# protolambda/go-kzg

Hardware: AMD Instinct MI355X
Metric: KZG commitments/sec (CommitToPoly, 4096-element blob); FK20 half: value_fk20_4096 (higher is better)
Workload: dtype u32; 1 GPU; CommitToPoly, 4096-coeff blobs, eth/trusted_setup.json monomial setup (s=1337), 4096 blobs/step/GPU resident in HBM, fixed-base table budget 110 GB (library default 110 GB: signed 16-bit windows, 8 of them walked by both GLV halves of every scalar, 103 GB; see table_sweep); global_batch=4096, parallelism=dp1 (independent blobs, no data-path collective)

## Files before the change

### go-kzg_amd/csrc/capi_common.hpp

```cpp
#pragma once
#include "../../include/kzg_hip.h"
#include "kzg_hip_internal.h"
#include "internal.hpp"
#include "fr_fft4096.hpp"
#include "fr_das2048.hpp"
#include "coalesce.hpp"
#include "sha256.hpp"

#include <algorithm>
#include <atomic>
#include <map>
#include <memory>
#include <mutex>
#include <shared_mutex>
#include <new>
#include <string>
#include <thread>
#include <chrono>
#include <condition_variable>
#include <vector>
#include <cstdio>
#include <cstring>
#include <cstdlib>

using namespace kzg;

extern thread_local std::string g_last_error;

#define HIPCHK(expr)                                                                                         \
    do {                                                                                                     \
        hipError_t e_ = (expr);                                                                              \
        if (e_ != hipSuccess) {                                                                              \
            char buf_[512];                                                                                  \
            snprintf(buf_, sizeof buf_, "%s failed: %s (%s:%d)", #expr, hipGetErrorString(e_), __FILE__, __LINE__); \
            g_last_error = buf_;                                                                             \
            (void)hipGetLastError();  \
            return KZG_HIP_ERR_HIP;                                                                          \
        }                                                                                                    \
    } while (0)
#define CHK(expr) do { int s_ = (expr); if (s_ != KZG_HIP_OK) return s_; } while (0)
#define KZG_TRY try {
#define KZG_CATCH                                                                                             \
    } catch (const std::bad_alloc &) { g_last_error = "host allocation failed"; return KZG_HIP_ERR_HIP; }    \
    catch (const std::exception &e_) { g_last_error = e_.what(); return KZG_HIP_ERR_HIP; }

inline bool is_pow2(uint64_t v) { return (v & (v - 1)) == 0; }
inline uint64_t next_pow2(uint64_t v) { if (v == 0) return 1; uint64_t p = 1; while (p < v) p <<= 1; return p; }

struct kzg_hip_fft {
    int device = 0;
    hipStream_t stream = nullptr;
    unsigned max_scale = 0;
    uint64_t W = 0;
    std::vector<fr> h_expanded, h_reversed;
    fr *d_expanded = nullptr, *d_reversed = nullptr;
    fr *d_expanded_l = nullptr, *d_reversed_l = nullptr;
    fr *d_inv_pow2 = nullptr;
    uint32_t *d_tw_das2048 = nullptr;
    uint32_t *d_tw4096[2] = {nullptr, nullptr};
    fr *d_glv_expanded = nullptr, *d_glv_reversed = nullptr;
    int8_t *d_wnaf_expanded = nullptr, *d_wnaf_reversed = nullptr;
    uint8_t *h_stage = nullptr; size_t h_stage_cap = 0;
    std::mutex mu;
    struct pool_slot { hipStream_t s = nullptr; uint8_t *h_pin = nullptr; size_t pin_cap = 0; };
    std::mutex pool_mu; std::condition_variable pool_cv; std::vector<pool_slot> pool_idle; int pool_total = 0;
    g2a *d_g2_fb = nullptr; uint64_t g2_fb_builds = 0;
    struct lincomb_promo *promo = nullptr;
};
struct g2_state;
struct kzg_hip_kzg {
    kzg_hip_fft *fs = nullptr;
    uint64_t n_setup = 0;
    g1j *d_secret = nullptr;
    g1a *d_secret_a = nullptr;
    g1a *d_fixed = nullptr;
    msm_plan fixed_plan{};
    double budget_gb = -1.0;
    std::atomic<bool> projective{false};
    hipStream_t copy_stream = nullptr;
    hipEvent_t copy_done[2] = {nullptr, nullptr};
    std::unique_ptr<coalescer> co_commit, co_proof;
    std::shared_ptr<g2_state> g2;
    std::mutex g2_mu;
    std::shared_mutex tab_mu;
};
struct fk20_core {
    kzg_hip_kzg *ks = nullptr;
    uint64_t n2 = 0, l = 1, k = 0;
    g1j *d_files = nullptr;
    g1a *d_files_fb = nullptr;
    uint32_t fb_c = 0, fb_nwin = 0; bool fb_glv = false;
    std::unique_ptr<coalescer> co_da;
};
struct kzg_hip_fk20s { fk20_core c; };
struct kzg_hip_fk20m { fk20_core c; };

struct dev_guard {
    kzg_hip_fft *fs; std::unique_lock<std::mutex> lk;
    explicit dev_guard(kzg_hip_fft *f) : fs(f), lk(f->mu) { hipSetDevice(f->device); }
};

struct dev_select { explicit dev_select(kzg_hip_fft *f) { hipSetDevice(f->device); } };
struct stream_lease {
    static constexpr int POOL_MAX = 16;
    static constexpr size_t PIN_MAX = 8u << 20;
    kzg_hip_fft *fs; hipStream_t s = nullptr; kzg_hip_fft::pool_slot slot; std::unique_lock<std::mutex> fallback;
    explicit stream_lease(kzg_hip_fft *f) : fs(f) {
        hipSetDevice(f->device);
        std::unique_lock<std::mutex> lk(f->pool_mu);
        for (;;) {
            if (!f->pool_idle.empty()) { slot = f->pool_idle.back(); f->pool_idle.pop_back(); s = slot.s; return; }
            if (f->pool_total < POOL_MAX) {
                if (hipStreamCreateWithFlags(&slot.s, hipStreamNonBlocking) == hipSuccess) { stream_cache_own(slot.s); f->pool_total++; s = slot.s; return; }
                (void)hipGetLastError(); slot.s = nullptr;
                if (f->pool_total == 0) { lk.unlock(); fallback = std::unique_lock<std::mutex>(f->mu); s = f->stream; return; }
            }
            f->pool_cv.wait(lk);
        }
    }
    stream_lease(kzg_hip_fft *f, std::try_to_lock_t) : fs(f) {
        std::unique_lock<std::mutex> lk(f->pool_mu);
        if (!f->pool_idle.empty()) { slot = f->pool_idle.back(); f->pool_idle.pop_back(); s = slot.s; return; }
        if (f->pool_total >= POOL_MAX) return;
        if (hipStreamCreateWithFlags(&slot.s, hipStreamNonBlocking) == hipSuccess) { stream_cache_own(slot.s); f->pool_total++; s = slot.s; return; }
        (void)hipGetLastError(); slot.s = nullptr;
    }
    uint8_t *pinned(size_t bytes, void **dev) {
        if (fallback.owns_lock() || bytes > PIN_MAX) return nullptr;
        if (slot.pin_cap < bytes) {
            if (slot.h_pin) { hipHostFree(slot.h_pin); slot.h_pin = nullptr; slot.pin_cap = 0; }
            size_t cap = bytes < (1u << 20) ? (1u << 20) : bytes;
            if (hipHostMalloc((void **)&slot.h_pin, cap, hipHostMallocDefault) != hipSuccess) { (void)hipGetLastError(); slot.h_pin = nullptr; return nullptr; }
            slot.pin_cap = cap;
        }
        if (hipHostGetDevicePointer(dev, slot.h_pin, 0) != hipSuccess) { (void)hipGetLastError(); return nullptr; }
        return slot.h_pin;
    }
    ~stream_lease() {
        if (!s) return;
        if (fallback.owns_lock()) { (void)hipStreamSynchronize(s); return; }
        (void)hipStreamSynchronize(slot.s);
        std::lock_guard<std::mutex> lk(fs->pool_mu);
        fs->pool_idle.push_back(slot);
        fs->pool_cv.notify_one();
    }
};
inline int d2h_staged(kzg_hip_fft *fs, hipStream_t s, void *host_dst, const void *dev_src, size_t bytes) {
    if (bytes > (16u << 20) || bytes < (1u << 20)) {
        HIPCHK(hipMemcpyAsync(host_dst, dev_src, bytes, hipMemcpyDeviceToHost, s));
        HIPCHK(hipStreamSynchronize(s));
        return KZG_HIP_OK;
    }
    if (fs->h_stage_cap < bytes) {
        if (fs->h_stage) { hipHostFree(fs->h_stage); fs->h_stage = nullptr; fs->h_stage_cap = 0; }
        size_t cap = 8u << 20;
        while (cap < bytes) cap <<= 1;
        if (hipHostMalloc((void **)&fs->h_stage, cap, hipHostMallocDefault) != hipSuccess) {
            (void)hipGetLastError(); fs->h_stage = nullptr;
            HIPCHK(hipMemcpyAsync(host_dst, dev_src, bytes, hipMemcpyDeviceToHost, s));
            HIPCHK(hipStreamSynchronize(s));
            return KZG_HIP_OK;
        }
        fs->h_stage_cap = cap;
    }
    HIPCHK(hipMemcpyAsync(fs->h_stage, dev_src, bytes, hipMemcpyDeviceToHost, s));
    HIPCHK(hipStreamSynchronize(s));
    memcpy(host_dst, fs->h_stage, bytes);
    return KZG_HIP_OK;
}
struct drain_on_exit {
    hipStream_t s;
    explicit drain_on_exit(hipStream_t st) : s(st) {}
    ~drain_on_exit() { (void)hipStreamSynchronize(s); }
};
void stream_cache_own(hipStream_t s);
void stream_cache_disown(hipStream_t s);
void *stream_cache_take(hipStream_t s, size_t class_bytes);
bool stream_cache_give(hipStream_t s, void *p, size_t class_bytes);
inline size_t stream_cache_class(size_t bytes) {
    if (bytes > (8u << 20)) return 0;
    size_t c = 256;
    while (c < bytes) c <<= 1;
    return c;
}
template <class T> struct dtmp {
    T *p = nullptr; hipStream_t s; size_t cls = 0;
    dtmp(hipStream_t st) : s(st) {}
    int alloc(size_t count) {
        if (!count) count = 1;
        size_t bytes = count * sizeof(T);
        cls = stream_cache_class(bytes);
        if (cls) {
            if ((p = (T *)stream_cache_take(s, cls))) return KZG_HIP_OK;
            bytes = cls;
        }
        HIPCHK(hipMallocAsync((void **)&p, bytes, s));
        return KZG_HIP_OK;
    }
    ~dtmp() { if (p && !(cls && stream_cache_give(s, p, cls))) hipFreeAsync(p, s); }
};


struct kzg_hip_points {
    kzg_hip_fft *fs = nullptr;
    uint64_t n = 0;
    g1a *d_tab = nullptr;
    kzg_hip_kzg *ks = nullptr;
    std::unique_ptr<coalescer> co;
};
struct kzg_hip_eth {
    kzg_hip_fft *fs = nullptr;
    kzg_hip_kzg *ks = nullptr;
    uint64_t n = 0;
    fr *d_domain = nullptr;
    std::unique_ptr<coalescer> co_blob;
    std::unique_ptr<coalescer> co_proof;
    std::shared_ptr<g2_state> g2;
    std::mutex g2_mu;
    std::vector<std::pair<hipEvent_t, std::shared_ptr<g2_state>>> g2_queued;
};

void fr_fft_rows(kzg_hip_fft *fs, hipStream_t s, const fr *d_in, uint64_t in_stride, uint64_t n_in, fr *d_out, uint64_t n, uint64_t batch, int inv);
uint32_t g1_fft_direct_logr(uint64_t n, uint64_t batch);
bool g1_fft_direct_mode(uint64_t n, uint64_t batch);
int g1_fft_direct_lanes(uint64_t n, uint64_t batch);
int g1_fft_rows(kzg_hip_fft *fs, hipStream_t s, const g1j *d_in, uint64_t in_stride, uint64_t n_valid, g1j *d_data, uint64_t n, uint64_t batch, int inv,
                           const fr *scale = nullptr, uint64_t n_out = 0);
int das_ext_rows(kzg_hip_fft *fs, hipStream_t s, fr *d, uint64_t n, uint64_t batch);
msm_plan classic_plan(uint64_t n, bool folded = false);
void set_inf_image(void *out_g1);
int kzg_settings_build(kzg_hip_fft *fs, const void *points_g1, uint64_t n, kzg_hip_kzg **out);
int ensure_fixed_table(kzg_hip_kzg *ks, hipStream_t);
const void *host_mapped_pointer(const void *host, size_t bytes);
int h2d_copy(void *dst, const void *src, size_t bytes, hipStream_t s);
int commit_rows(kzg_hip_kzg *ks, hipStream_t s, const fr *d_sc, uint64_t n, uint64_t batch, g1j *d_out, uint64_t sc_stride = 0, bool to_kilic = true);
double table_budget_gb(knobs::opt_gb env, double cap_gb, double headroom_gb);
int lincomb_points_rows(kzg_hip_points *pts, hipStream_t s, const fr *d_sc, uint64_t n, uint64_t batch, g1j *d_out, uint64_t sc_stride = 0, bool holds_mu = false);
int lincomb_points_coalesced(kzg_hip_points *pts, const void *scalars_fr, uint64_t n, void *out_g1);
uint32_t fb_windows(uint32_t c);
uint32_t fb_windows_glv(uint32_t c);
bool fb_glv_enabled();
bool coalescing_enabled();
coalescer *get_coalescer(kzg_hip_fft *fs, std::unique_ptr<coalescer> &slot, size_t in_row, size_t out_row, int callers_per_batch = 0);
int coalesce_upload_rows(coalesce_buf &b, uint64_t batch, size_t in_row_bytes, uint64_t n_max, fr *d_rows, uint64_t *d_meta);
int proof_single_rows(kzg_hip_kzg *ks, hipStream_t s, const fr *d_poly, uint64_t n, uint64_t batch, const uint64_t *d_x_u64, uint64_t x_stride, g1j *d_out);
int eth_g2_lines(kzg_hip_eth *eth, std::shared_ptr<g2_state> &hold, const g2_prepared **gen, const g2_prepared **s1);
int eth_g2_hold_on_stream(kzg_hip_eth *eth, hipStream_t s, const std::shared_ptr<g2_state> &hold);
void eth_g2_release_passed(kzg_hip_eth *eth, bool all = false);
int fk20_hext(fk20_core *c, hipStream_t s, const fr *d_poly, uint64_t poly_stride, uint64_t n, uint64_t batch, uint64_t j0, uint64_t cnt, g1j *d_hext);
int fk20_finish(fk20_core *c, hipStream_t s, const g1j *d_hext, uint64_t batch, int da, int bit_reverse, g1j *d_out);
int fk20_run_dev(fk20_core *c, hipStream_t s, const fr *d_poly, uint64_t poly_stride, uint64_t n, uint64_t batch, int da, int bit_reverse, g1j *d_out);
```

### go-kzg_amd/csrc/capi_kzg.hip

```cpp
#include "capi_common.hpp"

int kzg_settings_build(kzg_hip_fft *fs, const void *points_g1, uint64_t n, kzg_hip_kzg **out) {
    dev_guard g(fs);
    hipStream_t s = fs->stream;
    std::unique_ptr<kzg_hip_kzg, void (*)(kzg_hip_kzg *)> own(new kzg_hip_kzg, kzg_hip_kzg_settings_free);
    kzg_hip_kzg *ks = own.get();
    ks->fs = fs; ks->n_setup = n;
    dtmp<g1j> d_raw(s);
    CHK(d_raw.alloc(n));
    HIPCHK(hipMalloc((void **)&ks->d_secret, n * sizeof(g1j)));
    HIPCHK(hipMalloc((void **)&ks->d_secret_a, n * sizeof(g1a)));
    HIPCHK(hipMemcpyAsync(d_raw.p, points_g1, n * sizeof(g1j), hipMemcpyHostToDevice, s));
    launch_g1_from_kilic(s, d_raw.p, n);
    launch_g1_normalize(s, d_raw.p, ks->d_secret, n);
    launch_g1_to_affine(s, ks->d_secret, ks->d_secret_a, n);
    HIPCHK(hipGetLastError());
    HIPCHK(hipStreamSynchronize(s));
    *out = own.release();
    return KZG_HIP_OK;
}
int kzg_hip_kzg_settings_new(kzg_hip_fft *fs, const void *secret_g1, uint64_t n_setup, kzg_hip_kzg **out) {
    if (!fs || !out || !secret_g1) return KZG_HIP_ERR_BAD_ARG;
    *out = nullptr;
    if (n_setup < fs->W) return KZG_HIP_ERR_LEN_MISMATCH;
    KZG_TRY
    return kzg_settings_build(fs, secret_g1, n_setup, out);
    KZG_CATCH
}
void kzg_hip_kzg_settings_free(kzg_hip_kzg *ks) {
    if (!ks) return;
    hipSetDevice(ks->fs->device);
    hipDeviceSynchronize();
    hipFree(ks->d_secret); hipFree(ks->d_secret_a); hipFree(ks->d_fixed);
    if (ks->copy_stream) { stream_cache_disown(ks->copy_stream); hipStreamDestroy(ks->copy_stream); }
    for (int i = 0; i < 2; i++) if (ks->copy_done[i]) hipEventDestroy(ks->copy_done[i]);
    (void)hipGetLastError();
    delete ks;
}

double table_budget_gb(knobs::opt_gb env, double cap_gb, double headroom_gb) {
    if (env.set) return env.gb;
    size_t free_b = 0, total_b = 0;
    if (hipMemGetInfo(&free_b, &total_b) != hipSuccess) return 0.0;
    double g = (double)free_b / 1e9 - headroom_gb;
    return g > cap_gb ? cap_gb : (g > 0.0 ? g : 0.0);
}
uint32_t fb_windows(uint32_t c) {
    uint32_t nw = (255 + c - 1) / c, sh = c * (nw - 1);
    uint64_t top = (0x73eda753299d7d48ull >> (sh - 192)) + 1;
    return top > (1ull << (c - 1)) ? nw + 1 : nw;
}

#ifndef FB_DEFAULT_BUDGET_GB
#define FB_DEFAULT_BUDGET_GB 110.0
#endif
uint32_t fb_windows_glv(uint32_t c) { return (128 + c - 1) / c; }
bool fb_glv_enabled() { return knobs::fb_glv(); }
int ensure_fixed_table(kzg_hip_kzg *ks, hipStream_t) {
    if (ks->d_fixed || ks->fixed_plan.c == 0xffffffffu) return KZG_HIP_OK;
    hipStream_t s = ks->fs->stream;
    double budget_gb = ks->budget_gb >= 0.0 ? ks->budget_gb : table_budget_gb(knobs::fb_budget_gb(), FB_DEFAULT_BUDGET_GB, 24.0);
    if (ks->n_setup < 64) { ks->fixed_plan.c = 0xffffffffu; return KZG_HIP_OK; }
    const bool glv = fb_glv_enabled();
    for (uint32_t c = 16; c >= 5; c--) {
        if (glv ? (c == 14) : (c == 15)) continue;
        const uint32_t nwin = glv ? fb_windows_glv(c) : fb_windows(c);
        double bytes = (double)nwin * (double)ks->n_setup * (double)(1u << (c - 1)) * sizeof(g1a);
        if (bytes > budget_gb * 1e9) continue;
        msm_plan p{};
        p.c = c; p.nwin = nwin; p.nb = 1u << (c - 1); p.ngroups = 1; p.fixed = 1; p.glv = glv ? 1 : 0; p.table_n = ks->n_setup;
        size_t entries = (size_t)p.nwin * ks->n_setup * p.nb;
        g1a *tab = nullptr;
        if (hipMalloc((void **)&tab, entries * sizeof(g1a)) != hipSuccess) { (void)hipGetLastError(); continue; }
        hipError_t e = launch_fb_build(s, ks->d_secret_a, ks->n_setup, p.c, p.nwin, tab);
        if (e == hipSuccess) e = hipStreamSynchronize(s);
        if (e != hipSuccess) { (void)hipGetLastError(); hipFree(tab); continue; }
        ks->d_fixed = tab; ks->fixed_plan = p;
        return KZG_HIP_OK;
    }
    ks->fixed_plan.c = 0xffffffffu;
    return KZG_HIP_OK;
}

int commit_rows(kzg_hip_kzg *ks, hipStream_t s, const fr *d_sc, uint64_t n, uint64_t batch, g1j *d_out, uint64_t sc_stride, bool to_kilic) {
    CHK(ensure_fixed_table(ks, s));
    bool fixed = ks->d_fixed != nullptr;
    if (!sc_stride) sc_stride = n;
    msm_plan p = fixed ? ks->fixed_plan : classic_plan(ks->n_setup);
    if (!fixed && !msm_index_range_ok(p, n)) return KZG_HIP_ERR_TOO_WIDE;
    size_t ws_main = fixed ? fb_partials_bytes(n, batch) : msm_workspace_bytes(p, n, batch);
    dtmp<uint8_t> d_ws(s);
    CHK(d_ws.alloc(ws_main));
    if (fixed) launch_fb_msm(s, ks->d_fixed, p.table_n, p.c, p.nwin, d_sc, sc_stride, n, batch, d_ws.p, d_out, to_kilic, p.glv != 0, to_kilic && ks->projective.load(std::memory_order_relaxed));
    else launch_msm(s, p, ks->d_secret_a, d_sc, sc_stride, n, batch, d_ws.p, d_out, to_kilic);
    HIPCHK(hipGetLastError());
    return KZG_HIP_OK;
}
int kzg_hip_kzg_set_table_budget_gb(kzg_hip_kzg *ks, double gb) {
    if (!ks || !(gb >= 0.0)) return KZG_HIP_ERR_BAD_ARG;
    std::unique_lock<std::shared_mutex> tl(ks->tab_mu);
    dev_guard g(ks->fs);
    if (ks->d_fixed) { HIPCHK(hipDeviceSynchronize()); HIPCHK(hipFree(ks->d_fixed)); ks->d_fixed = nullptr; }
    ks->fixed_plan = msm_plan{};
    ks->budget_gb = gb;
    return KZG_HIP_OK;
}

int kzg_hip_commit_to_poly_batch_dev(kzg_hip_kzg *ks, const void *d_coeffs_fr, uint64_t n, uint64_t batch, void *d_out_g1, void *stream) {
    if (!ks || !d_out_g1) return KZG_HIP_ERR_BAD_ARG;
    if (n > ks->n_setup) return KZG_HIP_ERR_LEN_MISMATCH;
    if (!batch) return KZG_HIP_OK;
    if (n == 0 || !d_coeffs_fr) return KZG_HIP_ERR_BAD_ARG;
    dev_guard g(ks->fs);
    return commit_rows(ks, (hipStream_t)stream, (const fr *)d_coeffs_fr, n, batch, (g1j *)d_out_g1);
}
namespace {
std::mutex g_reg_mu;
std::map<uintptr_t, size_t> g_registered;
}
const void *host_mapped_pointer(const void *host, size_t bytes) {
    hipPointerAttribute_t a;
    if (hipPointerGetAttributes(&a, host) != hipSuccess) { (void)hipGetLastError(); return nullptr; }
    if (a.type != hipMemoryTypeHost || !a.devicePointer) return nullptr;
    const uintptr_t h = (uintptr_t)host;
    {
        std::lock_guard<std::mutex> lk(g_reg_mu);
        auto it = g_registered.upper_bound(h);
        if (it != g_registered.begin()) {
            --it;
            if (h >= it->first && h < it->first + it->second) return (h + bytes <= it->first + it->second) ? a.devicePointer : nullptr;
        }
    }
    hipDeviceptr_t base = nullptr; size_t size = 0;
    if (hipMemGetAddressRange(&base, &size, (hipDeviceptr_t)a.devicePointer) != hipSuccess) { (void)hipGetLastError(); return nullptr; }
    const uintptr_t d = (uintptr_t)a.devicePointer, b = (uintptr_t)base;
    return (d >= b && d + bytes <= b + size) ? a.devicePointer : nullptr;
}
int h2d_copy(void *dst, const void *src, size_t bytes, hipStream_t s) {
    uintptr_t p = (uintptr_t)src; uint8_t *d = (uint8_t *)dst;
    while (bytes) {
        size_t chunk = bytes;
        {
            std::lock_guard<std::mutex> lk(g_reg_mu);
            auto it = g_registered.upper_bound(p);
            if (it != g_registered.end() && it->first - p < chunk) chunk = it->first - p;
            if (it != g_registered.begin()) {
                --it;
                if (p < it->first + it->second && it->first + it->second - p < chunk) chunk = it->first + it->second - p;
            }
        }
        HIPCHK(hipMemcpyAsync(d, (const void *)p, chunk, hipMemcpyHostToDevice, s));
        p += chunk; d += chunk; bytes -= chunk;
    }
    return KZG_HIP_OK;
}
int kzg_hip_host_register(void *host, uint64_t bytes) {
    if (!host || !bytes) return KZG_HIP_ERR_BAD_ARG;
    KZG_TRY
    {
        std::lock_guard<std::mutex> lk(g_reg_mu);
        const uintptr_t h = (uintptr_t)host;
        auto it = g_registered.lower_bound(h);
        if (it != g_registered.end() && it->first < h + bytes) { g_last_error = "kzg_hip_host_register: the range overlaps a registered one (unregister it first)"; return KZG_HIP_ERR_BAD_ARG; }
        if (it != g_registered.begin()) { --it; if (it->first + it->second > h) { g_last_error = "kzg_hip_host_register: the range overlaps a registered one (unregister it first)"; return KZG_HIP_ERR_BAD_ARG; } }
    }
    HIPCHK(hipHostRegister(host, bytes, hipHostRegisterPortable | hipHostRegisterMapped));
    std::lock_guard<std::mutex> lk(g_reg_mu);
    g_registered[(uintptr_t)host] = bytes;
    return KZG_HIP_OK;
    KZG_CATCH
}
int kzg_hip_host_unregister(void *host) {
    if (!host) return KZG_HIP_ERR_BAD_ARG;
    KZG_TRY
    {
        std::lock_guard<std::mutex> lk(g_reg_mu);
        const uintptr_t h = (uintptr_t)host;
        auto it = g_registered.upper_bound(h);
        if (it != g_registered.begin()) {
            --it;
            if (h > it->first && h < it->first + it->second) { g_last_error = "kzg_hip_host_unregister: the address lies inside a registered range but is not its base"; return KZG_HIP_ERR_BAD_ARG; }
        }
    }
    HIPCHK(hipHostUnregister(host));
    std::lock_guard<std::mutex> lk(g_reg_mu);
    g_registered.erase((uintptr_t)host);
    return KZG_HIP_OK;
    KZG_CATCH
}
int kzg_hip_commit_to_poly_batch(kzg_hip_kzg *ks, const void *coeffs_fr, uint64_t n, uint64_t batch, void *out_g1) {
    if (!ks || !out_g1) return KZG_HIP_ERR_BAD_ARG;
    if (n > ks->n_setup) return KZG_HIP_ERR_LEN_MISMATCH;
    if (!batch) return KZG_HIP_OK;
    if (n == 0) { for (uint64_t b = 0; b < batch; b++) set_inf_image((uint8_t *)out_g1 + b * sizeof(g1j)); return KZG_HIP_OK; }
    if (!coeffs_fr) return KZG_HIP_ERR_BAD_ARG;
    dev_guard g(ks->fs);
    hipStream_t s = ks->fs->stream;
    dtmp<fr> d_sc(s); dtmp<g1j> d_out(s);
    CHK(d_out.alloc(batch));
    if (const fr *mapped = (const fr *)host_mapped_pointer(coeffs_fr, (size_t)n * batch * sizeof(fr))) {
        CHK(commit_rows(ks, s, mapped, n, batch, d_out.p));
        HIPCHK(hipMemcpyAsync(out_g1, d_out.p, batch * sizeof(g1j), hipMemcpyDeviceToHost, s));
        HIPCHK(hipStreamSynchronize(s));
        return KZG_HIP_OK;
    }
    CHK(d_sc.alloc(n * batch));
    uint64_t chunk = batch >= 1024 ? 512 : (batch >= 512 ? 256 : batch);
    if (chunk < batch && n * sizeof(fr) >= (64u << 10)) {
        if (!ks->copy_stream) {
            HIPCHK(hipStreamCreateWithFlags(&ks->copy_stream, hipStreamNonBlocking));
            stream_cache_own(ks->copy_stream);
            for (int i = 0; i < 2; i++) HIPCHK(hipEventCreateWithFlags(&ks->copy_done[i], hipEventDisableTiming));
        }
        CHK(ensure_fixed_table(ks, s));
        HIPCHK(hipStreamSynchronize(s));
        const bool ramp = knobs::upload_ramp() && batch >= 1024;
        int slot = 0;
        uint64_t step = 0;
        for (uint64_t b0 = 0, cnt = 0; b0 < batch; b0 += cnt, slot ^= 1, step++) {
            uint64_t want = chunk;
            if (ramp && step == 0) want = 64; else if (ramp && step == 1) want = 192;
            cnt = batch - b0 < want ? batch - b0 : want;
            CHK(h2d_copy(d_sc.p + b0 * n, (const fr *)coeffs_fr + b0 * n, n * cnt * sizeof(fr), ks->copy_stream));
            HIPCHK(hipEventRecord(ks->copy_done[slot], ks->copy_stream));
            HIPCHK(hipStreamWaitEvent(s, ks->copy_done[slot], 0));
            CHK(commit_rows(ks, s, d_sc.p + b0 * n, n, cnt, d_out.p + b0));
        }
    } else {
        CHK(h2d_copy(d_sc.p, coeffs_fr, n * batch * sizeof(fr), s));
        CHK(commit_rows(ks, s, d_sc.p, n, batch, d_out.p));
    }
    HIPCHK(hipMemcpyAsync(out_g1, d_out.p, batch * sizeof(g1j), hipMemcpyDeviceToHost, s));
    HIPCHK(hipStreamSynchronize(s));
    return KZG_HIP_OK;
}
bool coalescing_enabled() { return knobs::coalesce(); }
static uint64_t coalesce_rows(size_t in_row, size_t out_row) {
    size_t row = in_row > out_row ? in_row : out_row;
    uint64_t r = (64u << 20) / (row ? row : 1);
    return r < 4 ? 4 : (r > 256 ? 256 : r);
}
coalescer *get_coalescer(kzg_hip_fft *fs, std::unique_ptr<coalescer> &slot, size_t in_row, size_t out_row, int callers_per_batch) {
    std::lock_guard<std::mutex> lk(fs->mu);
    if (!slot) slot.reset(new coalescer(fs->device, in_row, out_row, coalesce_rows(in_row, out_row), callers_per_batch));
    return slot.get();
}
int coalesce_upload_rows(coalesce_buf &b, uint64_t batch, size_t in_row_bytes, uint64_t n_max, fr *d_rows, uint64_t *d_meta) {
    hipStream_t s = b.stream;
    HIPCHK(hipMemcpyAsync(d_meta, b.h_meta, batch * sizeof(coalesce_row), hipMemcpyHostToDevice, s));
    if (in_row_bytes == n_max * sizeof(fr)) HIPCHK(hipMemcpyAsync(d_rows, b.h_in, batch * in_row_bytes, hipMemcpyHostToDevice, s));
    else if (batch <= 4) { for (uint64_t r = 0; r < batch; r++) HIPCHK(hipMemcpyAsync(d_rows + r * n_max, b.h_in + r * in_row_bytes, n_max * sizeof(fr), hipMemcpyHostToDevice, s)); }
    else HIPCHK(hipMemcpy2DAsync(d_rows, n_max * sizeof(fr), b.h_in, in_row_bytes, n_max * sizeof(fr), batch, hipMemcpyHostToDevice, s));
    launch_fr_zero_tails(s, d_rows, n_max, batch, d_meta, 2);
    return KZG_HIP_OK;
}
int kzg_hip_commit_to_poly(kzg_hip_kzg *ks, const void *coeffs_fr, uint64_t n, void *out_g1) {
    if (!coalescing_enabled() || !ks || !out_g1 || !coeffs_fr || n == 0 || n > ks->n_setup)
        return kzg_hip_commit_to_poly_batch(ks, coeffs_fr, n, 1, out_g1);
    KZG_TRY
    coalescer *co = get_coalescer(ks->fs, ks->co_commit, ks->n_setup * sizeof(fr), sizeof(g1j));
    auto exec = [ks, co](coalesce_buf &b, uint64_t batch) -> int {
        hipSetDevice(ks->fs->device);
        hipStream_t s = b.stream;
        drain_on_exit drain(s);
        std::shared_lock<std::shared_mutex> tl(ks->tab_mu);
        { dev_guard g(ks->fs); CHK(ensure_fixed_table(ks, s)); }
        uint64_t n_max = 0;
        for (uint64_t i = 0; i < batch; i++) n_max = b.h_meta[i].n > n_max ? b.h_meta[i].n : n_max;
        dtmp<fr> d_rows(s); dtmp<uint64_t> d_meta(s);
        void *dp_out = nullptr;
        HIPCHK(hipHostGetDevicePointer(&dp_out, b.h_out, 0));
        g1j *d_out = (g1j *)dp_out;
        const bool trace = knobs::coalesce_trace();
        const auto t0 = std::chrono::steady_clock::now();
        bool uniform = ks->d_fixed != nullptr;
        for (uint64_t i = 0; i < batch && uniform; i++) uniform = b.h_meta[i].n == n_max;
        const fr *d_src = d_rows.p; uint64_t stride = n_max;
        if (uniform) {
            void *dp = nullptr;
            HIPCHK(hipHostGetDevicePointer(&dp, b.h_in, 0));
            d_src = (const fr *)dp; stride = co->in_row_bytes() / sizeof(fr);
        } else {
            CHK(d_rows.alloc(batch * n_max)); CHK(d_meta.alloc(2 * batch));
            d_src = d_rows.p;
            CHK(coalesce_upload_rows(b, batch, co->in_row_bytes(), n_max, d_rows.p, d_meta.p));
        }
        if (trace) hipStreamSynchronize(s);
        const auto t1 = std::chrono::steady_clock::now();
        CHK(commit_rows(ks, s, d_src, n_max, batch, d_out, stride));
        if (trace) hipStreamSynchronize(s);
        const auto t2 = std::chrono::steady_clock::now();
        HIPCHK(hipStreamSynchronize(s));
        if (trace) {
            auto us = [](std::chrono::steady_clock::time_point a, std::chrono::steady_clock::time_point c) { return std::chrono::duration<double, std::micro>(c - a).count(); };
            fprintf(stderr, "[commit batch %llu] upload %.0f us, kernels %.0f us, final synchronisation %.0f us\n", (unsigned long long)batch, us(t0, t1), us(t1, t2),
                    us(t2, std::chrono::steady_clock::now()));
        }
        return KZG_HIP_OK;
    };
    return co->submit(coeffs_fr, n * sizeof(fr), n, 0, out_g1, sizeof(g1j), exec, KZG_HIP_ERR_HIP);
    KZG_CATCH
}

int lincomb_points_coalesced(kzg_hip_points *pts, const void *scalars_fr, uint64_t n, void *out_g1) {
    if (!coalescing_enabled()) return kzg_hip_lincomb_points_batch(pts, scalars_fr, n, 1, out_g1);
    KZG_TRY
    coalescer *co = get_coalescer(pts->fs, pts->co, pts->n * sizeof(fr), sizeof(g1j));
    auto exec = [pts, co](coalesce_buf &b, uint64_t batch) -> int {
        hipSetDevice(pts->fs->device);
        hipStream_t s = b.stream;
        drain_on_exit drain(s);
        uint64_t n_max = 0;
        for (uint64_t i = 0; i < batch; i++) n_max = b.h_meta[i].n > n_max ? b.h_meta[i].n : n_max;
        bool uniform = true;
        for (uint64_t i = 0; i < batch && uniform; i++) uniform = b.h_meta[i].n == n_max;
        dtmp<fr> d_rows(s); dtmp<uint64_t> d_meta(s);
        void *dp_out = nullptr;
        HIPCHK(hipHostGetDevicePointer(&dp_out, b.h_out, 0));
        const fr *d_src; uint64_t stride;
        if (uniform) {
            void *dp = nullptr;
            HIPCHK(hipHostGetDevicePointer(&dp, b.h_in, 0));
            d_src = (const fr *)dp; stride = co->in_row_bytes() / sizeof(fr);
        } else {
            CHK(d_rows.alloc(batch * n_max)); CHK(d_meta.alloc(2 * batch));
            CHK(coalesce_upload_rows(b, batch, co->in_row_bytes(), n_max, d_rows.p, d_meta.p));
            d_src = d_rows.p; stride = n_max;
        }
        CHK(lincomb_points_rows(pts, s, d_src, n_max, batch, (g1j *)dp_out, stride));
        HIPCHK(hipStreamSynchronize(s));
        return KZG_HIP_OK;
    };
    return co->submit(scalars_fr, n * sizeof(fr), n, 0, out_g1, sizeof(g1j), exec, KZG_HIP_ERR_HIP);
    KZG_CATCH
}

int proof_single_rows(kzg_hip_kzg *ks, hipStream_t s, const fr *d_poly, uint64_t n, uint64_t batch, const uint64_t *d_x_u64, uint64_t x_stride, g1j *d_out) {
    dtmp<fr> d_q(s), d_x(s);
    CHK(d_q.alloc(batch * (n - 1))); CHK(d_x.alloc(batch));
    launch_fr_from_u64(s, d_x_u64, x_stride, d_x.p, batch);
    launch_quotient_linear(s, d_poly, n, n, batch, d_x.p, d_q.p, n - 1);
    return commit_rows(ks, s, d_q.p, n - 1, batch, d_out);
}
int kzg_hip_compute_proof_single_batch_dev(kzg_hip_kzg *ks, const void *d_poly_fr, uint64_t n, uint64_t batch, const void *d_x_u64, void *d_out_g1, void *stream) {
    if (!ks || !d_out_g1 || n < 2) return KZG_HIP_ERR_BAD_ARG;
    if (n - 1 > ks->n_setup) return KZG_HIP_ERR_LEN_MISMATCH;
    if (!batch) return KZG_HIP_OK;
    if (!d_poly_fr || !d_x_u64) return KZG_HIP_ERR_BAD_ARG;
    dev_guard g(ks->fs);
    return proof_single_rows(ks, (hipStream_t)stream, (const fr *)d_poly_fr, n, batch, (const uint64_t *)d_x_u64, 1, (g1j *)d_out_g1);
}
int kzg_hip_compute_proof_single_batch(kzg_hip_kzg *ks, const void *poly_fr, uint64_t n, uint64_t batch, const uint64_t *xs, void *out_g1) {
    if (!ks || !out_g1 || n < 2) return KZG_HIP_ERR_BAD_ARG;
    if (n - 1 > ks->n_setup) return KZG_HIP_ERR_LEN_MISMATCH;
    if (!batch) return KZG_HIP_OK;
    if (!poly_fr || !xs) return KZG_HIP_ERR_BAD_ARG;
    dev_guard g(ks->fs);
    hipStream_t s = ks->fs->stream;
    dtmp<fr> d_poly(s); dtmp<uint64_t> d_x(s); dtmp<g1j> d_out(s);
    CHK(d_poly.alloc(n * batch)); CHK(d_x.alloc(batch)); CHK(d_out.alloc(batch));
    HIPCHK(hipMemcpyAsync(d_poly.p, poly_fr, n * batch * sizeof(fr), hipMemcpyHostToDevice, s));
    HIPCHK(hipMemcpyAsync(d_x.p, xs, batch * sizeof(uint64_t), hipMemcpyHostToDevice, s));
    CHK(proof_single_rows(ks, s, d_poly.p, n, batch, d_x.p, 1, d_out.p));
    HIPCHK(hipMemcpyAsync(out_g1, d_out.p, batch * sizeof(g1j), hipMemcpyDeviceToHost, s));
    HIPCHK(hipStreamSynchronize(s));
    return KZG_HIP_OK;
}
int kzg_hip_compute_proof_single(kzg_hip_kzg *ks, const void *poly_fr, uint64_t n, uint64_t x, void *out_g1) {
    if (!ks || !poly_fr || !out_g1 || n < 2) return KZG_HIP_ERR_BAD_ARG;
    if (!coalescing_enabled() || n - 1 > ks->n_setup) return kzg_hip_compute_proof_single_batch(ks, poly_fr, n, 1, &x, out_g1);
    KZG_TRY
    coalescer *co = get_coalescer(ks->fs, ks->co_proof, (ks->n_setup + 1) * sizeof(fr), sizeof(g1j));
    auto exec = [ks, co](coalesce_buf &b, uint64_t batch) -> int {
        hipSetDevice(ks->fs->device);
        hipStream_t s = b.stream;
        drain_on_exit drain(s);
        std::shared_lock<std::shared_mutex> tl(ks->tab_mu);
        { dev_guard g(ks->fs); CHK(ensure_fixed_table(ks, s)); }
        uint64_t n_max = 0;
        for (uint64_t i = 0; i < batch; i++) n_max = b.h_meta[i].n > n_max ? b.h_meta[i].n : n_max;
        void *dp_out = nullptr;
        HIPCHK(hipHostGetDevicePointer(&dp_out, b.h_out, 0));
        if (batch == 1) {
            void *dp_in = nullptr, *dp_meta = nullptr;
            HIPCHK(hipHostGetDevicePointer(&dp_in, b.h_in, 0));
            HIPCHK(hipHostGetDevicePointer(&dp_meta, b.h_meta, 0));
            CHK(proof_single_rows(ks, s, (const fr *)dp_in, n_max, 1, (const uint64_t *)dp_meta + 1, 2, (g1j *)dp_out));
            HIPCHK(hipStreamSynchronize(s));
            return KZG_HIP_OK;
        }
        dtmp<fr> d_rows(s); dtmp<uint64_t> d_meta(s);
        CHK(d_rows.alloc(batch * n_max)); CHK(d_meta.alloc(2 * batch));
        CHK(coalesce_upload_rows(b, batch, co->in_row_bytes(), n_max, d_rows.p, d_meta.p));
        CHK(proof_single_rows(ks, s, d_rows.p, n_max, batch, d_meta.p + 1, 2, (g1j *)dp_out));
        HIPCHK(hipStreamSynchronize(s));
        return KZG_HIP_OK;
    };
    return co->submit(poly_fr, n * sizeof(fr), n, x, out_g1, sizeof(g1j), exec, KZG_HIP_ERR_HIP);
    KZG_CATCH
}

int kzg_hip_compute_proof_multi(kzg_hip_kzg *ks, const void *poly_fr, uint64_t len, uint64_t x, uint64_t n, void *out_g1) {
    (void)x;
    if (!ks || !poly_fr || !out_g1 || len < n + 1) return KZG_HIP_ERR_BAD_ARG;
    uint64_t nq = len - n;
    if (nq > ks->n_setup) return KZG_HIP_ERR_LEN_MISMATCH;
    return kzg_hip_commit_to_poly(ks, (const uint8_t *)poly_fr + n * sizeof(fr), nq, out_g1);
}
int kzg_hip_check_proof_multi_interpolation(kzg_hip_kzg *ks, const void *ys_fr, uint64_t n, const void *x_fr, void *out_is1_g1, void *out_xpow_fr) {
    if (!ks || !ys_fr || !x_fr || !out_is1_g1 || n == 0) return KZG_HIP_ERR_BAD_ARG;
    kzg_hip_fft *fs = ks->fs;
    if (n > fs->W) return KZG_HIP_ERR_TOO_WIDE;
    uint64_t np = next_pow2(n);
    if (np > ks->n_setup) return KZG_HIP_ERR_LEN_MISMATCH;
    dev_guard g(fs);
    hipStream_t s = fs->stream;
    dtmp<fr> d_ys(s), d_ip(s), d_x(s); dtmp<g1j> d_out(s);
    CHK(d_ys.alloc(n)); CHK(d_ip.alloc(np)); CHK(d_x.alloc(2)); CHK(d_out.alloc(1));
    HIPCHK(hipMemcpyAsync(d_ys.p, ys_fr, n * sizeof(fr), hipMemcpyHostToDevice, s));
    HIPCHK(hipMemcpyAsync(d_x.p, x_fr, sizeof(fr), hipMemcpyHostToDevice, s));
    fr_fft_rows(fs, s, d_ys.p, n, n, d_ip.p, np, 1, 1);
    launch_fr_scale_by_inv_powers(s, d_ip.p, d_x.p, np, d_x.p + 1);
    CHK(commit_rows(ks, s, d_ip.p, np, 1, d_out.p));
    HIPCHK(hipMemcpyAsync(out_is1_g1, d_out.p, sizeof(g1j), hipMemcpyDeviceToHost, s));
    if (out_xpow_fr) HIPCHK(hipMemcpyAsync(out_xpow_fr, d_x.p + 1, sizeof(fr), hipMemcpyDeviceToHost, s));
    HIPCHK(hipStreamSynchronize(s));
    return KZG_HIP_OK;
}
int kzg_hip_toeplitz_part2(kzg_hip_kzg *ks, const void *coeffs_fr, const void *x_ext_fft_g1, uint64_t n, void *out_g1) {
    if (!ks || !coeffs_fr || !x_ext_fft_g1 || !out_g1) return KZG_HIP_ERR_BAD_ARG;
    kzg_hip_fft *fs = ks->fs;
    if (n > fs->W) return KZG_HIP_ERR_TOO_WIDE;
    if (!is_pow2(n) || n == 0) return KZG_HIP_ERR_LEN_MISMATCH;
    stream_lease lease(fs);
    hipStream_t s = lease.s;
    dtmp<fr> d_c(s), d_cf(s); dtmp<g1j> d_x(s), d_h(s);
    CHK(d_c.alloc(n)); CHK(d_cf.alloc(n)); CHK(d_x.alloc(n)); CHK(d_h.alloc(n));
    HIPCHK(hipMemcpyAsync(d_c.p, coeffs_fr, n * sizeof(fr), hipMemcpyHostToDevice, s));
    HIPCHK(hipMemcpyAsync(d_x.p, x_ext_fft_g1, n * sizeof(g1j), hipMemcpyHostToDevice, s));
    launch_g1_from_kilic(s, d_x.p, n);
    fr_fft_rows(fs, s, d_c.p, n, n, d_cf.p, n, 1, 0);
    launch_g1_mul_vec(s, d_x.p, n, d_cf.p, 1, n, d_h.p);
    launch_g1_normalize(s, d_h.p, d_x.p, n, true);
    HIPCHK(hipGetLastError());
    HIPCHK(hipMemcpyAsync(out_g1, d_x.p, n * sizeof(g1j), hipMemcpyDeviceToHost, s));
    HIPCHK(hipStreamSynchronize(s));
    return KZG_HIP_OK;
}
int kzg_hip_toeplitz_part3(kzg_hip_kzg *ks, const void *h_ext_fft_g1, uint64_t n, void *out_g1) {
    if (!ks) return KZG_HIP_ERR_BAD_ARG;
    if (n > ks->fs->W) return KZG_HIP_ERR_TOO_WIDE;
    if (!is_pow2(n)) return KZG_HIP_ERR_NOT_POW2;
    if (n == 0 || !h_ext_fft_g1 || !out_g1) return KZG_HIP_ERR_BAD_ARG;
    KZG_TRY
    std::vector<g1j> full(n);
    CHK(kzg_hip_fft_g1(ks->fs, h_ext_fft_g1, n, 1, full.data()));
    memcpy(out_g1, full.data(), (n / 2) * sizeof(g1j));
    return KZG_HIP_OK;
    KZG_CATCH
}

int kzg_hip_kzg_table_info(kzg_hip_kzg *ks, uint32_t *window_bits, uint32_t *windows, uint64_t *table_bytes) {
    if (!ks || !window_bits || !windows || !table_bytes) return KZG_HIP_ERR_BAD_ARG;
    bool have = ks->d_fixed != nullptr;
    *window_bits = have ? ks->fixed_plan.c : 0; *windows = have ? ks->fixed_plan.nwin : 0;
    *table_bytes = have ? (uint64_t)ks->fixed_plan.nwin * ks->fixed_plan.table_n * ks->fixed_plan.nb * sizeof(g1a) : 0;
    return KZG_HIP_OK;
}
int kzg_hip_kzg_set_projective_outputs(kzg_hip_kzg *ks, int on) {
    if (!ks) return KZG_HIP_ERR_BAD_ARG;
    ks->projective.store(on != 0, std::memory_order_relaxed);
    return KZG_HIP_OK;
}
uint32_t kzg_hip_kzg_table_additions(kzg_hip_kzg *ks) {
    if (!ks || !ks->d_fixed) return 0;
    return ks->fixed_plan.glv ? 2 * ks->fixed_plan.nwin : ks->fixed_plan.nwin;
}
```

### go-kzg_amd/csrc/internal.hpp

```cpp
#pragma once
#include <hip/hip_runtime.h>
#include <stdint.h>
#include "field.hpp"
#include "g1.hpp"
#include "knobs.hpp"

namespace kzg {

inline uint32_t ilog2(uint64_t v) { uint32_t r = 0; while ((1ull << r) < v) r++; return r; }

void launch_fr_fft(hipStream_t s, const fr *in, uint64_t in_stride, uint64_t n_in, fr *out, uint64_t n, uint64_t batch,
                   const fr *roots, uint64_t W, const fr *scale, const uint32_t *tw4096 = nullptr, const fr *roots_l = nullptr);
bool fr_fft_lazy_sizes(uint64_t n, uint64_t batch);
void launch_das_ext(hipStream_t s, fr *vals, uint64_t n, uint64_t batch, const fr *expanded, const fr *reversed, uint64_t W,
                    const fr *inv_n, const uint32_t *tw2048 = nullptr);
void launch_toeplitz_coeffs(hipStream_t s, const fr *poly, uint64_t poly_stride, uint64_t n, uint64_t l, uint64_t batch, fr *out,
                            const fr *scale);
void launch_quotient_linear(hipStream_t s, const fr *poly, uint64_t poly_stride, uint64_t n, uint64_t batch, const fr *x, fr *q, uint64_t q_stride);
void launch_fr_from_u64(hipStream_t s, const uint64_t *in, uint64_t in_stride, fr *out, uint64_t n);
void launch_fr_zero_tails(hipStream_t s, fr *rows, uint64_t n_max, uint64_t batch, const uint64_t *lens, uint64_t lens_stride);
void launch_fr_any_nonzero(hipStream_t s, const fr *vals, uint64_t n, uint32_t *flag);
void launch_fr_powers(hipStream_t s, const fr *base, uint64_t n, fr *out);

void launch_fr_from_le32(hipStream_t s, const uint8_t *in, fr *out, uint64_t per_blob, uint64_t batch, uint32_t *bad);
void launch_fr_to_le32(hipStream_t s, const fr *in, uint8_t *out, uint64_t n);
void launch_fr_bitrev_gather(hipStream_t s, const fr *in, fr *out, uint64_t n);
constexpr uint64_t ZERO_TREE_LEAF = 16;
void launch_zero_leaves(hipStream_t s, const fr *expanded, uint64_t stride, const uint64_t *missing, uint64_t n_missing, uint64_t leaves, fr *a);
void launch_zero_pair_products(hipStream_t s, const fr *f, uint64_t m, uint64_t pairs, fr *out);
void launch_zero_join(hipStream_t s, fr *c, const fr *a, uint64_t d, uint64_t pairs);
void launch_zero_unpad(hipStream_t s, const fr *root, uint64_t pad, uint64_t n_missing, uint64_t length, fr *poly);
void launch_fr_mul_table_rows(hipStream_t s, fr *data, const fr *table, uint64_t stride, uint64_t n, uint64_t batch);
void launch_poly_lincomb(hipStream_t s, const fr *vectors, uint64_t stride, const fr *scalars, uint64_t count, uint64_t n, fr *out);
void launch_eth_quotient(hipStream_t s, const fr *poly, uint64_t poly_stride, const fr *domain, uint64_t n, uint64_t batch, const fr *z, uint64_t z_stride,
                         const fr *inv_n, fr *q, fr *y_out, uint32_t *flag, uint64_t dom_stride = 1, fr *scratch = nullptr);
uint64_t eth_quotient_scratch_elems(uint64_t n, uint64_t batch);

void launch_fr_scale_by_inv_powers(hipStream_t s, fr *c, const fr *x, uint64_t n, fr *xpow_n);

void launch_zero_eval_direct(hipStream_t s, const fr *expanded, uint64_t stride, const uint64_t *missing, uint64_t n_missing, uint64_t length, fr *zero_eval);
void launch_fr_scale_by_powers(hipStream_t s, fr *poly, const fr *base, uint64_t n);
void launch_fr_pointwise(hipStream_t s, const fr *a, const fr *b, const uint8_t *present, fr *out, uint64_t n, int mode, uint32_t *flag);
uint32_t launch_zero_eval_direct_rows_segs(uint64_t length, uint64_t rows, uint64_t nm_hint);
void launch_zero_eval_direct_rows(hipStream_t s, const fr *expanded, uint64_t stride, const uint64_t *missing, uint64_t list_stride, const uint64_t *n_missing, const fr *corr,
                                  uint32_t segs, uint64_t length, uint64_t rows, fr *zero_eval);

void launch_rr_scan(hipStream_t s, const uint8_t *present, uint64_t n, uint64_t rows, uint64_t *list, uint32_t *count, uint64_t *nm);
void launch_rr_corr(hipStream_t s, const uint64_t *nm, uint64_t rows, uint32_t segs, fr *corr);
void launch_rr_shift_bases(hipStream_t s, const fr &inv5, const fr &five, fr *out);
void launch_rr_leaves(hipStream_t s, const fr *expanded, uint64_t stride, const uint64_t *list, uint64_t list_stride, const uint64_t *nm, uint64_t leaves, uint64_t rows, fr *a);
void launch_rr_unpad(hipStream_t s, const fr *root, uint64_t leaves, const uint64_t *nm, uint64_t length, uint64_t rows, fr *poly);
void launch_rr_mask_mul(hipStream_t s, const fr *a, const fr *b, uint64_t b_stride, const uint8_t *present, uint64_t p_stride, uint64_t n, uint64_t rows, fr *out);
void launch_rr_strip_divide(hipStream_t s, const fr *num, const fr *den, fr *out, uint64_t total);
void launch_rr_finish(hipStream_t s, const fr *recon, const fr *samples, const uint8_t *present, uint64_t p_stride, const uint32_t *count, uint64_t c_stride, uint32_t *flag,
                      uint64_t n, uint64_t rows, fr *out, uint8_t *status);

void launch_g1_mul_vec(hipStream_t s, const g1j *pts, uint64_t pts_mod, const fr *scalars, uint64_t s_stride, uint64_t n, g1j *out);
hipError_t launch_g1_file_msm(hipStream_t s, const g1j *files, const fr *scalars, uint64_t nfiles, uint64_t k2, uint64_t j0, uint64_t cnt,
                              uint64_t batch, g1j *out);
void launch_g1_bitrev_copy(hipStream_t s, const g1j *in, uint64_t in_stride, uint64_t n_valid, g1j *out, uint64_t n, uint64_t batch);
void launch_g1_fft_stage(hipStream_t s, g1j *data, uint64_t n, uint64_t batch, uint64_t m, const fr *roots, const int8_t *wnaf, uint64_t W);
struct g1_stage_plan { int lanes; bool wnaf; bool rows; };
g1_stage_plan g1_fft_stage_plan(uint64_t n, uint64_t batch, uint64_t m, bool dif, int quad, knobs::g1_mul_mode mul);
g1_stage_plan g1_fft_stage_plan(uint64_t n, uint64_t batch, uint64_t m, bool dif);
void launch_g1_fft_stage_planned(hipStream_t s, const g1_stage_plan &plan, bool dif, g1j *data, uint64_t n, uint64_t batch, uint64_t m, const fr *roots, const int8_t *wnaf, uint64_t W);
void launch_g1_fft_stage_dif(hipStream_t s, g1j *data, uint64_t n, uint64_t batch, uint64_t m, const fr *roots, const int8_t *wnaf, uint64_t W);
void launch_g1_clear_odd(hipStream_t s, g1j *data, uint64_t n_total);
void launch_g1_take_even(hipStream_t s, const g1j *in, g1j *out, uint64_t total);
bool g1_quad_enabled();
void launch_fb_direct_pass1(hipStream_t s, const g1a *table, uint64_t table_n, uint32_t c, uint32_t nwin, const fr *scalars, const fr *roots, uint64_t W, uint64_t batch,
                            uint32_t logR, g1j *out, bool glv = false);
void launch_g1_stage_coop_dif(hipStream_t s, int lanes, bool wnaf_rows, g1j *data, uint64_t n, uint64_t batch, uint64_t m, const fr *roots, const int8_t *wnaf, uint64_t W, uint64_t total);
void launch_g1_stage_coop_dit(hipStream_t s, int lanes, bool wnaf_rows, g1j *data, uint64_t n, uint64_t batch, uint64_t m, const fr *roots, const int8_t *wnaf, uint64_t W, uint64_t total);
void launch_g1_direct_coop(hipStream_t s, int lanes, uint32_t wgs, size_t pad_lds, const g1j *src, uint64_t src_stride, uint64_t src_valid, g1j *dst, uint32_t logn, uint32_t logR,
                           uint64_t Ns, const fr *roots, uint64_t W, const fr *sc, uint64_t total, uint32_t logT, uint32_t logU);
void launch_g1_fft_direct(hipStream_t s, const g1j *in, uint64_t in_stride, uint64_t n_valid, g1j *data, g1j *tmp, uint64_t n, uint64_t batch, const fr *roots,
                          uint64_t W, const fr *scale, uint32_t max_logr = 4, int lanes = 1, uint32_t bits_done = 0, uint64_t n_out = 0,
                          bool lanes_fixed = false);
void launch_g1_normalize(hipStream_t s, const g1j *in, g1j *out, uint64_t n, bool to_kilic = false);
void launch_fr_inv_test(hipStream_t s, const fr *in, uint64_t n, fr *out_coop, fr *out_lane, fr *out_block);
void launch_fp_inv_both(hipStream_t s, const fp *in, fp *out_coop, fp *out_lane, uint64_t n, int mode);
void launch_g1_from_kilic(hipStream_t s, g1j *data, uint64_t n);
void launch_g1_to_affine(hipStream_t s, const g1j *in, g1a *out, uint64_t n);
void launch_g1_compress(hipStream_t s, const g1j *in, uint8_t *out48, uint64_t n);
void launch_g1_decompress(hipStream_t s, const uint8_t *in48, g1j *out, uint64_t n, uint32_t *bad_flag);
void launch_g1_fixed_base_powers(hipStream_t s, const fr *powers, uint64_t n, g1j *out);

uint64_t device_simd_lanes();
inline uint64_t device_simds() { return device_simd_lanes() / 64; }
struct msm_plan {
    uint32_t c;
    uint32_t nwin;
    uint32_t nb;
    uint32_t ngroups;
    uint32_t fixed;
    uint32_t glv;
    uint64_t table_n;
};
inline bool msm_index_range_ok(const msm_plan &p, uint64_t n) { return n < (1ull << 27) && 2 * p.table_n < (1ull << 30); }
size_t msm_workspace_bytes(const msm_plan &p, uint64_t n, uint64_t batch);
void launch_msm(hipStream_t s, const msm_plan &p, const g1a *table, const fr *scalars, uint64_t sc_stride, uint64_t n, uint64_t batch, void *workspace, g1j *out,
                bool to_kilic, uint64_t table_stride = 0, bool crowded_buckets = false);
void launch_msm_window_table(hipStream_t s, const g1a *pts, uint64_t n, uint32_t c, uint32_t nwin, g1j *tmp, g1a *out);

size_t fb_partials_bytes(uint64_t n, uint64_t batch);
hipError_t launch_fb_build(hipStream_t s, const g1a *pts, uint64_t n, uint32_t c, uint32_t nwin, g1a *table);
void launch_fb_msm(hipStream_t s, const g1a *table, uint64_t table_n, uint32_t c, uint32_t nwin, const fr *scalars, uint64_t sc_stride, uint64_t n,
                   uint64_t batch, void *partials, g1j *out, bool to_kilic, bool glv = false, bool projective = false);

void launch_fb_mul_vec(hipStream_t s, const g1a *table, uint64_t table_n, uint32_t c, uint32_t nwin, const fr *scalars, uint64_t row, uint64_t j0,
                       uint64_t cnt, uint64_t batch, g1j *out, bool glv = false);
void launch_fb_mul_vec_dif2(hipStream_t s, const g1a *table, uint64_t table_n, uint32_t c, uint32_t nwin, const fr *scalars, const fr *roots, uint64_t W,
                            uint64_t batch, g1j *out, bool glv = false);
void launch_fb_mul_vec_files(hipStream_t s, const g1a *table, uint64_t table_n, uint32_t c, uint32_t nwin, const fr *scalars, uint64_t row, uint64_t j0,
                             uint64_t cnt, uint64_t batch, g1j *out, bool glv = false);
void launch_g1_sum_files(hipStream_t s, const g1j *tmp, uint64_t nfiles, uint64_t cnt, uint64_t batch, g1j *out);

struct g2j; struct g2_prepared;
void launch_g2_from_compressed(hipStream_t s, const uint8_t *in96, g2j *out_kilic, uint64_t n, uint32_t *bad_flag);
void launch_g2_prepare(hipStream_t s, const g2j *in_kilic, uint64_t n, g2_prepared *out);
void launch_pairs_g1_from_kilic(hipStream_t s, const g1j *a1, const g1j *b1, uint64_t n, g1j *p0, g1j *p1);
void launch_kzg_check_inputs(hipStream_t s, const g1j *c, const g1j *pi, const fr *ys, const g1j *es, const fr *bs, uint64_t n, g1j *p0, g1j *p1);
void launch_fr_rows_scale_by_inv_powers(hipStream_t s, fr *c, uint64_t np, const fr *xs, uint64_t count, fr *xpow_n);
void launch_eth_check_inputs(hipStream_t s, const uint8_t *c48, const uint8_t *zs, const uint8_t *ys, const uint8_t *pi48, uint64_t n, g1j *p0, g1j *p1, uint8_t *status);
void launch_pairing_check(hipStream_t s, bool shared_lines, const g2_prepared *q0, const g2_prepared *q1, const g1j *p0, const g1j *p1, uint64_t n, uint8_t *ok);
void launch_pairing_value(hipStream_t s, const g1j *g1_kilic, const g2_prepared *q, uint64_t n, fp *out);
bool pairing_route_is_wave(uint64_t n);

constexpr uint64_t PAIRING_WAVE_BELOW = 16385;
void launch_pairing_check_wave(hipStream_t s, bool shared_lines, const g2_prepared *q0, const g2_prepared *q1, const g1j *p0, const g1j *p1, uint64_t n, uint8_t *ok);
void launch_pairing_value_wave(hipStream_t s, const g1j *g1_kilic, const g2_prepared *q, uint64_t n, fp *out);
void launch_wave_fp12_op(hipStream_t s, int op, const fp *a, const fp *b, uint64_t n, fp *out);

struct g2a;
void launch_g2_fixed_base_table(hipStream_t s, g2a *table);
void launch_g2_fixed_base(hipStream_t s, const fr *scalars, uint64_t n, const g2a *table, g2j *out);
void launch_g2_normalize(hipStream_t s, const g2j *in, uint64_t n, g2j *out_kilic);
void launch_g2_compress(hipStream_t s, const g2j *in_kilic, uint64_t n, uint8_t *out96);

void launch_eth_transcripts(hipStream_t s, const uint8_t *blobs, const uint8_t *comms, const uint64_t *off, uint64_t n, uint64_t sidecars, fr *r_out, fr *z_out);
void launch_eth_transcript_blobs(hipStream_t s, const uint8_t *blobs, const uint64_t *off, uint64_t n, uint64_t sidecars, uint32_t *st);
void launch_eth_transcript_finish(hipStream_t s, const uint8_t *blobs, const uint8_t *comms, const uint64_t *off, uint64_t n, uint64_t sidecars, const uint32_t *st,
                                  fr *r_out, fr *z_out);
void launch_eth_prove_finish(hipStream_t s, const uint8_t *agg_status, const uint32_t *z_in_domain, const uint64_t *off, uint64_t sidecars, uint8_t code_blob,
                             uint8_t code_z, uint8_t *proofs48, uint8_t *comms48, uint8_t *status);
void launch_eth_agg_poly(hipStream_t s, const uint8_t *blobs, const uint64_t *off, const fr *r, uint64_t n, uint64_t sidecars, fr *agg, uint8_t *status);
void launch_eth_powers(hipStream_t s, const fr *r, const uint64_t *off, uint64_t sidecars, fr *pow);
void launch_g1_decompress_rows(hipStream_t s, const uint8_t *in48, g1j *out, uint64_t n, uint8_t *bad, bool to_kilic);
void launch_g1_segment_sum(hipStream_t s, const g1j *pts, const uint8_t *pt_bad, const uint64_t *off, uint64_t sidecars, g1j *out, g1j *out_kilic, uint8_t *status);
void launch_eth_agg_finish(hipStream_t s, const uint32_t *z_in_domain, const uint8_t *proof_bad, uint64_t sidecars, fr *y, uint8_t *status);
void launch_test_sha256_lanes(hipStream_t s, const uint8_t *data, const uint64_t *offsets, const uint64_t *lens, uint64_t rows, uint32_t *out);
void launch_test_hash_to_bls_field_lanes(hipStream_t s, const uint8_t *digests, uint64_t rows, fr *out);

void launch_eth_versioned_hashes(hipStream_t s, const uint8_t *c48, uint64_t n, uint8_t *out32);
void launch_eth_precompile_inputs(hipStream_t s, const uint8_t *in192, uint64_t n, g1j *p0, g1j *p1, uint8_t *status);
void launch_eth_merge_status(hipStream_t s, const uint8_t *status, const uint8_t *ok, uint64_t n, uint8_t *result);
void launch_eth_tx_hashes_check(hipStream_t s, const uint8_t *c48, const uint8_t *want32, const uint64_t *off, uint64_t total, uint64_t blocks, uint8_t *match,
                                uint8_t *result);

struct combine_seed;
void launch_combine_scalars(hipStream_t s, const combine_seed &seed, const fr *xs, const fr *ys, const uint8_t *status, uint64_t row0, uint64_t count, uint64_t R, fr *sc);
void launch_combine_points(hipStream_t s, const g1j *c, const g1j *pi, uint64_t count, uint64_t R, bool kilic, g1j *out, const g1j *last = nullptr);
void launch_combine_negate(hipStream_t s, const g1j *a, uint64_t n, g1j *out);
void launch_eth_combine_fields(hipStream_t s, const uint8_t *zs, const uint8_t *ys, const uint8_t *c_bad, const uint8_t *pi_bad, uint64_t n, fr *z_out, fr *y_out,
                               uint8_t *status);

void launch_combine_multi_scalars(hipStream_t s, const combine_seed &seed, const fr *xs, const fr *coef, uint64_t np, uint64_t row0, uint64_t count, uint64_t R, fr *sc,
                                  fr *partials, fr *J);

void prof_begin(hipStream_t s, const char *name);
void prof_end(hipStream_t s, const char *name);

}
```

### go-kzg_amd/csrc/k_msm.hip

```cpp
#include "internal.hpp"
#include "g1_quad.hpp"
#include "coop_inv.hpp"
#include <atomic>
#include <cstring>

namespace kzg {

#define MSM_SORT_T 1024
#define MSM_ACC_BLOCK 128
#define MSM_NB 128

struct fb_partial { uint32_t w[52]; uint32_t inf; };
__device__ __forceinline__ void fb_partial_store(fb_partial &o, const g1x_acc &a) {
#pragma unroll
    for (int i = 0; i < 13; i++) { o.w[i] = a.v.x.l[i]; o.w[13 + i] = a.v.y.l[i]; o.w[26 + i] = a.v.zz.l[i]; o.w[39 + i] = a.v.zzz.l[i]; }
    o.inf = a.inf ? 1u : 0u;
}
__device__ __forceinline__ void fb_partial_load(const fb_partial &p, g1xq &v) {
#pragma unroll
    for (int i = 0; i < 13; i++) { v.x.l[i] = p.w[i]; v.y.l[i] = p.w[13 + i]; v.zz.l[i] = p.w[26 + i]; v.zzz.l[i] = p.w[39 + i]; }
}

template <uint32_t DELTA> __device__ __forceinline__ uint32_t lane_down(uint32_t v) {
    if constexpr (DELTA < 16) return (uint32_t)__builtin_amdgcn_update_dpp((int)v, (int)v, 0x100 + DELTA, 0xf, 0xf, false);
    else return (uint32_t)__builtin_amdgcn_ds_bpermute((int)((((threadIdx.x & 63u) + DELTA) & 63u) << 2), (int)v);
}
template <uint32_t DELTA> __device__ __forceinline__ void point_down(g1xq &o, uint32_t &oinf, const g1xq &v, uint32_t vinf) {
#pragma unroll
    for (int i = 0; i < 13; i++) {
        o.x.l[i] = lane_down<DELTA>(v.x.l[i]); o.y.l[i] = lane_down<DELTA>(v.y.l[i]);
        o.zz.l[i] = lane_down<DELTA>(v.zz.l[i]); o.zzz.l[i] = lane_down<DELTA>(v.zzz.l[i]);
    }
    oinf = lane_down<DELTA>(vinf);
}
__device__ __forceinline__ void point_down_any(g1xq &o, uint32_t &oinf, const g1xq &v, uint32_t vinf, uint32_t off) {
    switch (off) {
    case 4: point_down<4>(o, oinf, v, vinf); break;
    case 8: point_down<8>(o, oinf, v, vinf); break;
    case 16: point_down<16>(o, oinf, v, vinf); break;
    default: point_down<32>(o, oinf, v, vinf); break;
    }
}

#ifndef MSM_SEG
#define MSM_SEG 64
#endif
struct msm_ws_layout {
    size_t entries_off, offsets_off, buckets_off, gsum_off, segs_off, per_blob;
    uint64_t K, nent, nseg;
};
static msm_ws_layout ws_layout(const msm_plan &p, uint64_t n) {
    msm_ws_layout L;
    L.K = (uint64_t)p.ngroups * MSM_NB;
    L.nent = n * 32;
    size_t o = 0;
    L.entries_off = o; o += ((L.nent * 4 + 15) / 16) * 16;
    L.offsets_off = o; o += (((2 * L.K + 1) * 4 + 15) / 16) * 16;
    L.buckets_off = o; o += ((L.K * sizeof(fb_partial) + 15) / 16) * 16;
    L.gsum_off = o; o += (((size_t)p.ngroups * sizeof(fb_partial) + 15) / 16) * 16;
    L.nseg = (L.nent + MSM_SEG - 1) / MSM_SEG;
    L.segs_off = o; o += ((L.nseg * 2 * sizeof(fb_partial) + 15) / 16) * 16;
    L.per_blob = o;
    return L;
}
size_t msm_workspace_bytes(const msm_plan &p, uint64_t n, uint64_t batch) { return ws_layout(p, n).per_blob * batch; }

template <class Fn> __device__ __forceinline__ void for_each_glv_digit(const fr &k_mont, Fn f) {
    const glv_halves h = glv_split_signed(from_mont<FrP>(k_mont));
#pragma unroll
    for (uint32_t half = 0; half < 2; half++) {
        const uint32_t *mag = half ? h.k2 : h.k1;
        const uint32_t sgn = half ? h.neg2 : h.neg1;
        uint32_t carry = 0;
#pragma unroll
        for (uint32_t w = 0; w < 16; w++) {
            uint32_t raw = ((mag[w >> 2] >> ((w & 3) * 8)) & 255u) + carry;
            if (raw > MSM_NB) { carry = 1; f(w, 256u - raw, half, sgn ^ 1u); }
            else { carry = 0; f(w, raw, half, sgn); }
        }
    }
}

__global__ __launch_bounds__(MSM_SORT_T) void k_msm_sort(uint32_t ngroups, uint64_t table_n, const fr *scalars, uint64_t sc_stride, uint64_t n, uint8_t *ws,
                                                         size_t per_blob, size_t entries_off, size_t offsets_off, uint32_t K) {
    extern __shared__ uint32_t smem[];
    uint32_t *hist = smem, *part = smem + K;
    const uint32_t tid = threadIdx.x;
    const uint64_t b = blockIdx.x;
    const fr *sc = scalars + b * sc_stride;
    uint32_t *entries = (uint32_t *)(ws + b * per_blob + entries_off);
    uint32_t *offsets = (uint32_t *)(ws + b * per_blob + offsets_off);
    const uint32_t wmask = ngroups - 1;
    for (uint32_t i = tid; i < K; i += MSM_SORT_T) hist[i] = 0;
    __syncthreads();
    for (uint64_t i = tid; i < n; i += MSM_SORT_T)
        for_each_glv_digit(sc[i], [&](uint32_t w, uint32_t mag, uint32_t half, uint32_t) {
            if (mag) atomicAdd(&hist[(((w & wmask) * MSM_NB + mag - 1) << 1) | (half ^ 1u)], 1u);
        });
    __syncthreads();
    const uint32_t per = (K + MSM_SORT_T - 1) / MSM_SORT_T;
    uint32_t lo = tid * per, hi = lo + per < K ? lo + per : K, sum = 0;
    for (uint32_t i = lo; i < hi; i++) sum += hist[i];
    part[tid] = sum;
    __syncthreads();
    for (uint32_t off = 1; off < MSM_SORT_T; off <<= 1) {
        uint32_t v = tid >= off ? part[tid - off] : 0;
        __syncthreads();
        part[tid] += v;
        __syncthreads();
    }
    uint32_t run = part[tid] - sum;
    for (uint32_t i = lo; i < hi; i++) { uint32_t cnt = hist[i]; offsets[i] = run; hist[i] = run; run += cnt; }
    if (tid == MSM_SORT_T - 1) offsets[K] = part[tid];
    __syncthreads();
    for (uint64_t i = tid; i < n; i += MSM_SORT_T)
        for_each_glv_digit(sc[i], [&](uint32_t w, uint32_t mag, uint32_t half, uint32_t neg) {
            if (!mag) return;
            uint32_t slot = atomicAdd(&hist[(((w & wmask) * MSM_NB + mag - 1) << 1) | (half ^ 1u)], 1u);
            uint32_t pidx = (uint32_t)i + ((w & ~wmask) ? (uint32_t)table_n : 0u);
            entries[slot] = (pidx << 2) | (half << 1) | neg;
        });
}

__global__ __launch_bounds__(MSM_ACC_BLOCK, 2) void k_msm_accumulate(const g1a *table, uint64_t table_stride, uint8_t *ws, size_t per_blob, size_t entries_off, size_t offsets_off,
                                                                  size_t buckets_off, uint32_t K, uint32_t S, uint64_t total) {
    __shared__ fb_partial buf[MSM_ACC_BLOCK];
    const uint32_t tid = threadIdx.x;
    uint64_t t = blockIdx.x * (uint64_t)blockDim.x + tid;
    const bool live = t < total;
    const uint32_t sidx = (uint32_t)(t % S);
    const uint64_t bk = t / S;
    const uint64_t b = bk / K; const uint32_t key = (uint32_t)(bk % K);
    g1x_acc acc; acc.init();
    if (live) {
        const uint32_t *entries = (const uint32_t *)(ws + b * per_blob + entries_off);
        const uint32_t *offsets = (const uint32_t *)(ws + b * per_blob + offsets_off);
        const uint32_t s0 = offsets[2 * key], len = offsets[2 * key + 2] - s0;
        table += b * table_stride;
        const uint32_t s = s0 + (uint32_t)((uint64_t)len * sidx / S), e = s0 + (uint32_t)((uint64_t)len * (sidx + 1) / S);
#pragma nounroll
        for (uint32_t i = s; i < e; i++) {
            const uint32_t en = entries[i];
            g1a q = table[en >> 2];
            if (en & 2u) q.x = mul(q.x, glv_beta());
            if (en & 1u) q.y = neg<FpP>(q.y);
            acc.add(q);
        }
    }
    if (S > 1) {
        fb_partial_store(buf[tid], acc);
        __syncthreads();
#pragma nounroll
        for (uint32_t off = S / 2; off >= 1; off >>= 1) {
            if (sidx < off) {
                g1xq v; fb_partial_load(buf[tid + off], v);
                g1x_acc_merge(acc, v, buf[tid + off].inf != 0);
                fb_partial_store(buf[tid], acc);
            }
            __syncthreads();
        }
    }
    if (live && sidx == 0) fb_partial_store(((fb_partial *)(ws + b * per_blob + buckets_off))[key], acc);
}

__device__ __forceinline__ void acc_apply_phi(g1x_acc &a) { if (!a.inf) a.v.x = mulq(a.v.x, unpackq(glv_beta())); }
__global__ __launch_bounds__(MSM_ACC_BLOCK, 2) void k_msm_accumulate_seg(const g1a *table, uint64_t table_stride, uint8_t *ws, size_t per_blob, size_t entries_off, size_t offsets_off,
                                                                      size_t buckets_off, size_t segs_off, uint32_t K2, uint64_t nseg, uint64_t total) {
    const uint64_t t = blockIdx.x * (uint64_t)blockDim.x + threadIdx.x;
    if (t >= total) return;
    const uint64_t b = t / nseg; const uint32_t seg = (uint32_t)(t % nseg);
    table += b * table_stride;
    const uint32_t *entries = (const uint32_t *)(ws + b * per_blob + entries_off);
    const uint32_t *offsets = (const uint32_t *)(ws + b * per_blob + offsets_off);
    fb_partial *buckets = (fb_partial *)(ws + b * per_blob + buckets_off);
    fb_partial *slots = (fb_partial *)(ws + b * per_blob + segs_off) + 2ull * seg;
    const uint32_t E = offsets[K2];
    const uint32_t s = seg * MSM_SEG, e = s + MSM_SEG < E ? s + MSM_SEG : E;
    if (s >= e) return;
    uint32_t lo = 0, hi = K2;
    while (hi - lo > 1) { const uint32_t mid = (lo + hi) >> 1; if (offsets[mid] <= s) lo = mid; else hi = mid; }
    uint32_t key = lo, kend = offsets[key + 1];
    const uint32_t first_bucket = key >> 1;
    const bool first_open = offsets[key & ~1u] < s;
    g1x_acc acc; acc.init();
    uint32_t en_next = entries[s];
    g1a qn = table[en_next >> 2];
#pragma nounroll
    for (uint32_t i = s; i < e; i++) {
        while (i >= kend) {
            if (!(key & 1u)) acc_apply_phi(acc);
            if (key & 1u) {
                const uint32_t bk = key >> 1;
                if (bk == first_bucket && first_open) fb_partial_store(slots[0], acc); else fb_partial_store(buckets[bk], acc);
                acc.init();
            }
            key++; kend = offsets[key + 1];
        }
        g1a q = qn; const uint32_t en = en_next;
        if (i + 1 < e) { en_next = entries[i + 1]; qn = table[en_next >> 2]; }
        if (en & 1u) q.y = neg<FpP>(q.y);
        acc.add(q);
    }
    if (!(key & 1u)) acc_apply_phi(acc);
    const uint32_t bk = key >> 1;
    const bool last_closed = offsets[2 * bk + 2] <= e;
    if (bk == first_bucket) { if (!first_open && last_closed) fb_partial_store(buckets[bk], acc); else fb_partial_store(slots[0], acc); }
    else if (last_closed) fb_partial_store(buckets[bk], acc);
    else fb_partial_store(slots[1], acc);
}
__global__ __launch_bounds__(MSM_ACC_BLOCK, 2) void k_msm_merge_segs(uint8_t *ws, size_t per_blob, size_t offsets_off, size_t buckets_off, size_t segs_off, uint32_t K, uint64_t total) {
    const uint64_t t = blockIdx.x * (uint64_t)blockDim.x + threadIdx.x;
    if (t >= total) return;
    const uint64_t b = t / K; const uint32_t bk = (uint32_t)(t % K);
    const uint32_t *offsets = (const uint32_t *)(ws + b * per_blob + offsets_off);
    fb_partial *buckets = (fb_partial *)(ws + b * per_blob + buckets_off);
    const fb_partial *slots = (const fb_partial *)(ws + b * per_blob + segs_off);
    const uint32_t a = offsets[2 * bk], z = offsets[2 * bk + 2];
    g1x_acc acc; acc.init();
    if (a == z) { fb_partial_store(buckets[bk], acc); return; }
    const uint32_t seg_lo = a / MSM_SEG, seg_hi = (z - 1) / MSM_SEG;
    if (seg_lo == seg_hi) return;
#pragma nounroll
    for (uint32_t sg = seg_lo; sg <= seg_hi; sg++) {
        const fb_partial &p = slots[2ull * sg + ((sg == seg_lo && a > seg_lo * MSM_SEG) ? 1 : 0)];
        g1xq v; fb_partial_load(p, v);
        g1x_acc_merge(acc, v, p.inf != 0);
    }
    fb_partial_store(buckets[bk], acc);
}

__global__ __launch_bounds__(MSM_NB) void k_msm_reduce(uint8_t *ws, size_t per_blob, size_t buckets_off, size_t gsum_off, uint32_t ngroups) {
    __shared__ fb_partial buf[MSM_NB];
    const uint32_t d = threadIdx.x;
    const uint64_t b = blockIdx.x / ngroups; const uint32_t g = blockIdx.x % ngroups;
    const fb_partial *buckets = (const fb_partial *)(ws + b * per_blob + buckets_off) + (uint64_t)g * MSM_NB;
    g1x_acc acc; acc.inf = buckets[d].inf != 0;
    if (!acc.inf) fb_partial_load(buckets[d], acc.v);
    fb_partial_store(buf[d], acc);
    __syncthreads();
#pragma nounroll
    for (uint32_t off = 1; off < MSM_NB; off <<= 1) {
        g1xq v; bool vinf = true;
        if (d + off < MSM_NB) { vinf = buf[d + off].inf != 0; if (!vinf) fb_partial_load(buf[d + off], v); }
        __syncthreads();
        if (!vinf) { g1x_acc_merge(acc, v, false); fb_partial_store(buf[d], acc); }
        __syncthreads();
    }
#pragma nounroll
    for (uint32_t off = MSM_NB / 2; off >= 1; off >>= 1) {
        if (d < off) {
            g1xq v; fb_partial_load(buf[d + off], v);
            g1x_acc_merge(acc, v, buf[d + off].inf != 0);
            fb_partial_store(buf[d], acc);
        }
        __syncthreads();
    }
    if (d == 0) fb_partial_store(((fb_partial *)(ws + b * per_blob + gsum_off))[g], acc);
}

__device__ __forceinline__ void g1xq_dbl_lane(g1xq &p) {
    const fq u = addq(p.y, p.y);
    const fq v = sqrq(u), xx = sqrq(p.x);
    const fq m = addq(addq(xx, xx), xx);
    const fq w = mulq(u, v), s_ = mulq(p.x, v), zz3 = mulq(v, p.zz), mm = sqrq(m);
    const fq x3 = subq<5>(mm, addq(s_, s_));
    const fq t1 = mulq(m, subq<8>(s_, x3)), t2 = mulq(w, p.y), zzz3 = mulq(w, p.zzz);
    p.x = x3; p.y = subq<3>(t1, t2); p.zz = zz3; p.zzz = zzz3;
}
__global__ __launch_bounds__(MSM_NB) void k_msm_reduce_chunks(uint8_t *ws, size_t per_blob, size_t buckets_off, size_t gsum_off, uint32_t ngroups, uint64_t total_groups) {
    __shared__ fb_partial buf[MSM_NB];
    const uint32_t tid = threadIdx.x, c = tid & 31u;
    const uint64_t G = blockIdx.x * 4ull + (tid >> 5);
    const bool live = G < total_groups;
    const uint64_t b = live ? G / ngroups : 0; const uint32_t g = live ? (uint32_t)(G % ngroups) : 0;
    const fb_partial *buckets = (const fb_partial *)(ws + b * per_blob + buckets_off) + (uint64_t)g * MSM_NB + 4u * c;
    g1x_acc T, S; T.init(); S.init();
    if (live) {
#pragma nounroll
        for (int j = 3; j >= 0; j--) {
            const bool vinf = buckets[j].inf != 0;
            g1xq v;
            if (!vinf) { fb_partial_load(buckets[j], v); g1x_acc_merge(T, v, false); }
            if (!T.inf) { const g1xq t = T.v; g1x_acc_merge(S, t, false); }
        }
    }
    fb_partial_store(buf[tid], T);
    __syncthreads();
#pragma nounroll
    for (uint32_t off = 1; off < 32; off <<= 1) {
        g1xq v; bool vinf = true;
        if (c + off < 32) { vinf = buf[tid + off].inf != 0; if (!vinf) fb_partial_load(buf[tid + off], v); }
        __syncthreads();
        if (!vinf) { g1x_acc_merge(T, v, false); fb_partial_store(buf[tid], T); }
        __syncthreads();
    }
    if (c >= 1 && !T.inf) {
        g1xq q = T.v;
        g1xq_dbl_lane(q); g1xq_dbl_lane(q);
        g1x_acc_merge(S, q, false);
    }
    fb_partial_store(buf[tid], S);
    __syncthreads();
#pragma nounroll
    for (uint32_t off = 16; off >= 1; off >>= 1) {
        if (c < off) {
            g1xq v; fb_partial_load(buf[tid + off], v);
            g1x_acc_merge(S, v, buf[tid + off].inf != 0);
            fb_partial_store(buf[tid], S);
        }
        __syncthreads();
    }
    if (live && c == 0) fb_partial_store(((fb_partial *)(ws + b * per_blob + gsum_off))[g], S);
}

__global__ __launch_bounds__(256) void k_msm_combine(uint8_t *ws, size_t per_blob, size_t gsum_off, uint32_t ngroups, uint64_t batch, g1j *out, int to_kilic) {
    const uint32_t role = threadIdx.x & 3u;
    const uint64_t b = blockIdx.x * 64ull + (threadIdx.x >> 2);
    const bool live = b < batch;
    const fb_partial *gsum = (const fb_partial *)(ws + (live ? b : 0) * per_blob + gsum_off);
    g1x_acc acc; acc.init();
    acc.v = g1xq_from_affine(g1a_inf());
#pragma nounroll
    for (uint32_t g = ngroups; g-- > 0;) {
#pragma nounroll
        for (uint32_t j = 0; j < 8; j++) {
            g1xq d = acc.v;
            quad_xyzz_dbl(d, role);
            if (!acc.inf) acc.v = d;
        }
        const bool winf = !live || gsum[g].inf != 0;
        g1xq w;
        if (winf) w = acc.v; else fb_partial_load(gsum[g], w);
        quad_acc_add(acc, w, winf, role);
    }
    {
        const bool own = live && role == 0;
        const g1x px = g1xq_pack(acc.v);
        const fp i = wave_inv_any(mul(px.zz, px.zzz), own && !acc.inf);
        if (own) {
            g1j r;
            if (acc.inf) r = g1_inf();
            else { r.x = mul(px.x, mul(i, px.zzz)); r.y = mul(px.y, mul(i, px.zz)); r.z = one<FpP>(); }
            out[b] = to_kilic ? g1_to_kilic(r) : r;
        }
    }
}

void launch_msm(hipStream_t s, const msm_plan &p, const g1a *table, const fr *scalars, uint64_t sc_stride, uint64_t n, uint64_t batch, void *workspace, g1j *out,
                bool to_kilic, uint64_t table_stride, bool crowded_buckets) {
    if (!batch) return;
    msm_ws_layout L = ws_layout(p, n);
    uint8_t *ws = (uint8_t *)workspace;
    uint32_t K = (uint32_t)L.K;
    const uint32_t K2 = 2 * K;
    size_t sh = (size_t)(K2 + MSM_SORT_T) * 4;
    hipLaunchKernelGGL(k_msm_sort, dim3((uint32_t)batch), dim3(MSM_SORT_T), sh, s, p.ngroups, p.table_n, scalars, sc_stride, n, ws, L.per_blob, L.entries_off,
                       L.offsets_off, K2);
    uint32_t S = 1;
    while (S < 16 && batch * L.K * S * 2 <= 2 * device_simd_lanes()) S *= 2;
    uint64_t total = batch * L.K * S;
    const int seg_mode = knobs::msm_seg();
    prof_begin(s, "msm_accumulate");
    const bool balanced = seg_mode == 1 || (seg_mode < 0 && (batch * L.nseg >= 2 * device_simd_lanes() || (crowded_buckets && S < 8)));
    if (balanced) {
        const uint64_t tseg = batch * L.nseg, tb = batch * L.K;
        hipLaunchKernelGGL(k_msm_accumulate_seg, dim3((uint32_t)((tseg + MSM_ACC_BLOCK - 1) / MSM_ACC_BLOCK)), dim3(MSM_ACC_BLOCK), 0, s, table, table_stride, ws, L.per_blob,
                           L.entries_off, L.offsets_off, L.buckets_off, L.segs_off, K2, L.nseg, tseg);
        hipLaunchKernelGGL(k_msm_merge_segs, dim3((uint32_t)((tb + MSM_ACC_BLOCK - 1) / MSM_ACC_BLOCK)), dim3(MSM_ACC_BLOCK), 0, s, ws, L.per_blob, L.offsets_off,
                           L.buckets_off, L.segs_off, K, tb);
    } else
        hipLaunchKernelGGL(k_msm_accumulate, dim3((uint32_t)((total + MSM_ACC_BLOCK - 1) / MSM_ACC_BLOCK)), dim3(MSM_ACC_BLOCK), 0, s, table, table_stride, ws, L.per_blob,
                           L.entries_off, L.offsets_off, L.buckets_off, K, S, total);
    prof_end(s, "msm_accumulate");
    const knobs::msm_reduce_mode reduce_mode = knobs::msm_reduce();
    if (reduce_mode == knobs::msm_reduce_mode::chunks || (reduce_mode == knobs::msm_reduce_mode::by_batch && balanced && batch * p.ngroups * 32 >= device_simd_lanes())) {
        const uint64_t tg = batch * p.ngroups;
        hipLaunchKernelGGL(k_msm_reduce_chunks, dim3((uint32_t)((tg + 3) / 4)), dim3(MSM_NB), 0, s, ws, L.per_blob, L.buckets_off, L.gsum_off, p.ngroups, tg);
    } else
        hipLaunchKernelGGL(k_msm_reduce, dim3((uint32_t)(batch * p.ngroups)), dim3(MSM_NB), 0, s, ws, L.per_blob, L.buckets_off, L.gsum_off, p.ngroups);
    hipLaunchKernelGGL(k_msm_combine, dim3((uint32_t)((batch + 63) / 64)), dim3(256), 0, s, ws, L.per_blob, L.gsum_off, p.ngroups, batch, out, to_kilic ? 1 : 0);
}

#ifndef FB_BLOCK
#define FB_BLOCK 128
#endif
#ifndef FB_FINISH_LANES_MAX
#define FB_FINISH_LANES_MAX 4
#endif
#ifndef FB_KEEP
#define FB_KEEP 16
#endif
#ifndef FB_ACC_WAVES
#define FB_ACC_WAVES 2
#endif

__global__ __launch_bounds__(FB_BLOCK, 2) void k_fb_build_pass1(const g1a *rows, uint64_t lanes, uint32_t D, uint32_t S, g1a *table, fp *ztmp) {
    uint64_t t = blockIdx.x * (uint64_t)blockDim.x + threadIdx.x;
    const uint32_t segs = D / S;
    if (t >= lanes * segs) return;
    const uint64_t row = t / segs; const uint32_t seg = (uint32_t)(t % segs);
    g1a b = rows[row];
    g1j cur = to_jac(b);
    uint32_t k = seg * S + 1;
    if (k > 1) {
        cur = g1_inf();
#pragma nounroll
        for (int bit = 31 - __builtin_clz(k); bit >= 0; bit--) {
            cur = g1_dbl(cur);
            if ((k >> bit) & 1u) cur = g1_madd(cur, b);
        }
    }
    g1a *dst = table + row * D + (uint64_t)seg * S; fp *zd = ztmp + row * D + (uint64_t)seg * S;
#pragma nounroll
    for (uint32_t d = 0; d < S; d++) {
        g1a xy; xy.x = cur.x; xy.y = cur.y;
        dst[d] = xy; zd[d] = cur.z;
        cur = g1_madd(cur, b);
    }
}
__global__ __launch_bounds__(FB_BLOCK, 2) void k_fb_build_pass2(uint64_t lanes, uint32_t D, uint32_t S, g1a *table, fp *ztmp, fp *ptmp) {
    uint64_t t = blockIdx.x * (uint64_t)blockDim.x + threadIdx.x;
    if (t >= lanes * (D / S)) return;
    g1a *dst = table + t * S; fp *zd = ztmp + t * S; fp *pd = ptmp + t * S;
    fp acc = one<FpP>();
#pragma nounroll
    for (uint32_t d = 0; d < S; d++) {
        pd[d] = acc;
        fp z = zd[d];
        if (!is_zero<FpP>(z)) acc = mul(acc, z);
    }
    fp inv_all = inv<FpP>(acc);
#pragma nounroll
    for (uint32_t d = S; d-- > 0;) {
        fp z = zd[d];
        if (is_zero<FpP>(z)) { dst[d] = g1a_inf(); continue; }
        fp zi = mul(inv_all, pd[d]);
        inv_all = mul(inv_all, z);
        fp zi2 = sqr(zi);
        g1a xy = dst[d];
        xy.x = mul(xy.x, zi2); xy.y = mul(xy.y, mul(zi2, zi));
        dst[d] = xy;
    }
}

__device__ __forceinline__ void quad_tree_add(g1x_acc &acc, const g1xq &w, bool winf, uint32_t role) { quad_acc_add(acc, w, winf, role); }
template <int R> __device__ __forceinline__ void quad_point_bcast(g1xq &o, uint32_t &oinf, const g1xq &v, uint32_t vinf) {
    o.x = quad_bcast<R>(v.x); o.y = quad_bcast<R>(v.y); o.zz = quad_bcast<R>(v.zz); o.zzz = quad_bcast<R>(v.zzz);
    oinf = (uint32_t)__builtin_amdgcn_update_dpp((int)vinf, (int)vinf, R * 0x55, 0xf, 0xf, false);
}
__device__ __forceinline__ void quad_tree_reduce(g1x_acc &col, fb_partial *buf, uint32_t tid, uint32_t live) {
    const uint32_t role = tid & 3u, quad = tid >> 2;
    uint32_t off = 1;
    while (off < live) off *= 2;
#pragma nounroll
    for (off >>= 1; off >= 16; off >>= 1) {
        if (quad >= off && quad < 2 * off && role == 0) fb_partial_store(buf[quad], col);
        __syncthreads();
        if (quad < off) {
            const bool have = quad + off < live;
            const fb_partial &src = buf[have ? quad + off : off];
            g1xq w; fb_partial_load(src, w);
            quad_tree_add(col, w, !have || src.inf != 0, role);
        }
    }
    if (tid < 64) {
#pragma nounroll
        for (; off >= 1; off >>= 1) {
            const bool have = quad < off && quad + off < live;
            g1xq w; uint32_t wi;
            point_down_any(w, wi, col.v, col.inf ? 1u : 0u, 4 * off);
            quad_tree_add(col, w, !have || wi != 0, role);
        }
    }
}
__device__ __forceinline__ void fb_block_reduce_quad(g1x_acc &acc, fb_partial *buf, uint32_t tid) {
    const uint32_t role = tid & 3u;
    if (acc.inf) acc.v = g1xq_from_affine(g1a_inf());
    const uint32_t ainf = acc.inf ? 1u : 0u;
    g1x_acc col;
    { uint32_t vi; quad_point_bcast<0>(col.v, vi, acc.v, ainf); col.inf = vi != 0; }
    { g1xq v; uint32_t vi; quad_point_bcast<1>(v, vi, acc.v, ainf); quad_tree_add(col, v, vi != 0, role); }
    { g1xq v; uint32_t vi; quad_point_bcast<2>(v, vi, acc.v, ainf); quad_tree_add(col, v, vi != 0, role); }
    { g1xq v; uint32_t vi; quad_point_bcast<3>(v, vi, acc.v, ainf); quad_tree_add(col, v, vi != 0, role); }
    quad_tree_reduce(col, buf, tid, 64);
    acc = col;
}

#define FB_ACC_BLOCK 256
__device__ __forceinline__ uint32_t scalar_bits(const fr &k, uint32_t off, uint32_t c) {
    uint32_t idx = off >> 5, sh = off & 31;
    if (idx >= 8) return 0;
    uint64_t v = k.l[idx];
    if (idx + 1 < 8) v |= (uint64_t)k.l[idx + 1] << 32;
    return (uint32_t)(v >> sh) & ((1u << c) - 1u);
}

template <bool SPLIT> __global__ __launch_bounds__(FB_ACC_BLOCK, FB_ACC_WAVES) void k_fb_accumulate(const g1a *table, uint64_t table_n, uint32_t c, uint32_t nwin, uint32_t D, const fr *scalars,
                                                            uint64_t sc_stride, uint64_t n, uint32_t blocks_per_blob, uint32_t wsplit, fb_partial *partials) {
    __shared__ fb_partial buf[64];
    const uint32_t tid = threadIdx.x;
    const uint64_t blob = blockIdx.x / blocks_per_blob; const uint32_t blk = blockIdx.x % blocks_per_blob;
    const uint64_t L = (uint64_t)blocks_per_blob * FB_ACC_BLOCK;
    const fr *sc = scalars + blob * sc_stride;
    g1x_acc acc; acc.init();
    const uint32_t wpg = SPLIT ? (nwin + wsplit - 1) / wsplit : nwin;
    const uint64_t nv = SPLIT ? n * wsplit : n;
    for (uint64_t v = (uint64_t)blk * FB_ACC_BLOCK + tid; v < nv; v += L) {
        const uint64_t i = SPLIT ? v % n : v;
        const uint32_t w0 = SPLIT ? (uint32_t)(v / n) * wpg : 0u;
        const uint32_t w1 = SPLIT ? (w0 + wpg < nwin ? w0 + wpg : nwin) : nwin;
        if (SPLIT && w0 >= w1) continue;
        fr k = from_mont<FrP>(sc[i]);
        uint32_t raw, carry = 0, mag, ng;
        if (SPLIT) {
#pragma nounroll
            for (uint32_t w = 0; w < w0; w++) carry = (scalar_bits(k, w * c, c) + carry > D) ? 1u : 0u;
        }
        raw = scalar_bits(k, w0 * c, c) + carry;
        if (raw > D) { carry = 1; mag = (1u << c) - raw; ng = 1; } else { carry = 0; mag = raw; ng = 0; }
        g1a qn = table[((uint64_t)w0 * table_n + i) * D + (mag ? mag - 1 : 0)];
#pragma nounroll
        for (uint32_t w = w0; w < w1; w++) {
            g1a q = qn;
            const uint32_t cmag = mag, cng = ng;
            if (w + 1 < w1) {
                raw = scalar_bits(k, (w + 1) * c, c) + carry;
                if (raw > D) { carry = 1; mag = (1u << c) - raw; ng = 1; } else { carry = 0; mag = raw; ng = 0; }
                qn = table[((uint64_t)(w + 1) * table_n + i) * D + (mag ? mag - 1 : 0)];
            }
            if (cmag) {
                if (cng) q.y = neg<FpP>(q.y);
                acc.add(q);
            }
        }
    }
    fb_block_reduce_quad(acc, buf, tid);
    if (tid == 0) fb_partial_store(partials[blockIdx.x], acc);
}
__device__ __forceinline__ uint32_t mag_bits(const uint32_t (&m)[4], uint32_t off, uint32_t c) {
    const uint32_t idx = off >> 5, sh = off & 31;
    if (idx >= 4) return 0;
    uint64_t v = m[idx];
    if (idx + 1 < 4) v |= (uint64_t)m[idx + 1] << 32;
    return (uint32_t)(v >> sh) & ((1u << c) - 1u);
}
template <bool SPLIT> __global__ __launch_bounds__(FB_ACC_BLOCK, FB_ACC_WAVES) void k_fb_accumulate_glv(const g1a *table, uint64_t table_n, uint32_t c, uint32_t nwin, uint32_t D, const fr *scalars,
                                                            uint64_t sc_stride, uint64_t n, uint32_t blocks_per_blob, uint32_t wsplit, fb_partial *partials) {
    __shared__ fb_partial buf[64];
    const uint32_t tid = threadIdx.x;
    const uint64_t blob = blockIdx.x / blocks_per_blob; const uint32_t blk = blockIdx.x % blocks_per_blob;
    const uint64_t L = (uint64_t)blocks_per_blob * FB_ACC_BLOCK;
    const fr *sc = scalars + blob * sc_stride;
    g1x_acc acc; acc.init();
    const uint32_t wpg = SPLIT ? (nwin + wsplit - 1) / wsplit : nwin;
    const uint64_t nvh = SPLIT ? n * wsplit : n;
    bool in_phi = false;
    const bool keep_ok = !SPLIT && nvh % L == 0 && nvh / L <= FB_KEEP;
    uint32_t kept[FB_KEEP][5];
    uint32_t slot = 0;
    for (uint64_t v = (uint64_t)blk * FB_ACC_BLOCK + tid; v < 2 * nvh; v += L) {
        const bool phi = v < nvh;
        const uint64_t vh = phi ? v : v - nvh;
        const uint64_t i = SPLIT ? vh % n : vh;
        const uint32_t w0 = SPLIT ? (uint32_t)(vh / n) * wpg : 0u;
        const uint32_t w1 = SPLIT ? (w0 + wpg < nwin ? w0 + wpg : nwin) : nwin;
        if (SPLIT && w0 >= w1) continue;
        if (in_phi && !phi) { if (!acc.inf) acc.v.x = mulq(acc.v.x, unpackq(glv_beta())); in_phi = false; }
        uint32_t m[4], sgn;
        if (keep_ok && !phi) {
            const uint32_t at = slot < FB_KEEP ? slot : 0; slot++;
#pragma unroll
            for (int j = 0; j < 4; j++) m[j] = kept[at][j];
            sgn = kept[at][4];
            if (slot == (uint32_t)(nvh / L)) slot = 0;
        } else {
            const glv_halves h = glv_split_signed(from_mont<FrP>(sc[i]));
#pragma unroll
            for (int j = 0; j < 4; j++) m[j] = phi ? h.k2[j] : h.k1[j];
            sgn = phi ? h.neg2 : h.neg1;
            if (keep_ok) {
                const uint32_t at = slot < FB_KEEP ? slot : 0; slot++;
#pragma unroll
                for (int j = 0; j < 4; j++) kept[at][j] = h.k1[j];
                kept[at][4] = h.neg1;
                if (slot == (uint32_t)(nvh / L)) slot = 0;
            }
        }
        uint32_t raw, carry = 0, mag, ng;
        if (SPLIT) {
#pragma nounroll
            for (uint32_t w = 0; w < w0; w++) carry = (mag_bits(m, w * c, c) + carry > D) ? 1u : 0u;
        }
        raw = mag_bits(m, w0 * c, c) + carry;
        if (raw > D) { carry = 1; mag = (1u << c) - raw; ng = 1; } else { carry = 0; mag = raw; ng = 0; }
        g1a qn = table[((uint64_t)w0 * table_n + i) * D + (mag ? mag - 1 : 0)];
#pragma nounroll
        for (uint32_t w = w0; w < w1; w++) {
            g1a q = qn;
            const uint32_t cmag = mag, cng = ng;
            if (w + 1 < w1) {
                raw = mag_bits(m, (w + 1) * c, c) + carry;
                if (raw > D) { carry = 1; mag = (1u << c) - raw; ng = 1; } else { carry = 0; mag = raw; ng = 0; }
                qn = table[((uint64_t)(w + 1) * table_n + i) * D + (mag ? mag - 1 : 0)];
            }
            if (cmag) {
                if (cng ^ sgn) q.y = neg<FpP>(q.y);
                acc.add(q);
                in_phi = phi;
            }
        }
    }
    if (in_phi && !acc.inf) acc.v.x = mulq(acc.v.x, unpackq(glv_beta()));
    fb_block_reduce_quad(acc, buf, tid);
    if (tid == 0) fb_partial_store(partials[blockIdx.x], acc);
}
__global__ __launch_bounds__(256) void k_fb_finish(const fb_partial *partials, uint32_t blocks_per_blob, uint64_t batch, g1j *out, int to_kilic) {
    __shared__ fb_partial buf[64];
    const uint64_t b = blockIdx.x;
    const uint32_t tid = threadIdx.x, role = tid & 3u, quad = tid >> 2, col = tid & 63u;
    g1x_acc acc; acc.init();
    acc.v = g1xq_from_affine(g1a_inf());
    const uint32_t rounds = (blocks_per_blob + 63) / 64;
    g1xq wn; bool wn_inf;
    { const bool have = quad < blocks_per_blob; const fb_partial &pj = partials[b * blocks_per_blob + (have ? quad : 0)]; fb_partial_load(pj, wn); wn_inf = !have || pj.inf != 0; }
#pragma nounroll
    for (uint32_t r = 0; r < rounds; r++) {
        const g1xq w = wn; const bool winf = wn_inf;
        if (r + 1 < rounds) {
            const uint32_t j = (r + 1) * 64 + quad;
            const bool have = j < blocks_per_blob;
            const fb_partial &pj = partials[b * blocks_per_blob + (have ? j : 0)];
            fb_partial_load(pj, wn); wn_inf = !have || pj.inf != 0;
        }
        quad_tree_add(acc, w, winf, role);
    }
    quad_tree_reduce(acc, buf, tid, blocks_per_blob < 64 ? blocks_per_blob : 64);
    const bool first_wave = tid < 64;
    if (first_wave) {
        const bool own = col == 0;
        const g1x px = g1xq_pack(acc.v);
        const bool need = own && !acc.inf && !(to_kilic & 2);
        const fp i = wave_inv_any(mul(px.zz, px.zzz), need);
        const uint32_t aff = __builtin_amdgcn_readfirstlane((uint32_t)(!acc.inf && !(to_kilic & 2)));
        if (aff) {
            fp i1;
#pragma unroll
            for (int k = 0; k < 12; k++) i1.l[k] = (uint32_t)__builtin_amdgcn_readlane((int)i.l[k], 0);
            if (tid < 2) {
                fp c = mul(tid ? px.y : px.x, mul(i1, tid ? px.zz : px.zzz));
                if (to_kilic & 1) c = fp_to_kilic(c);
                fp *dst = tid ? &out[b].y : &out[b].x;
                *dst = c;
                if (tid == 0) out[b].z = (to_kilic & 1) ? fp_kilic_one() : one<FpP>();
            }
        } else if (own) {
            g1j r;
            if (acc.inf) r = g1_inf(); else r = g1x_to_jac(px);
            out[b] = (to_kilic & 1) ? g1_to_kilic(r) : r;
        }
    }
}

__global__ __launch_bounds__(64) void k_fb_finish_lanes(const fb_partial *partials, uint32_t blocks_per_blob, uint64_t batch, g1j *out, int to_kilic) {
    const uint64_t b = blockIdx.x * (uint64_t)blockDim.x + threadIdx.x;
    if (b >= batch) return;
    g1x_acc acc; acc.init();
#pragma nounroll
    for (uint32_t j = 0; j < blocks_per_blob; j++) {
        const fb_partial &pj = partials[b * blocks_per_blob + j];
        g1xq w; fb_partial_load(pj, w);
        g1x_acc_merge(acc, w, pj.inf != 0);
    }
    g1j r;
    if (acc.inf) r = g1_inf();
    else if (to_kilic & 2) r = g1x_to_jac(g1xq_pack(acc.v));
    else {
        g1x px = g1xq_pack(acc.v);
        fp i = inv<FpP>(mul(px.zz, px.zzz));
        r.x = mul(px.x, mul(i, px.zzz)); r.y = mul(px.y, mul(i, px.zz)); r.z = one<FpP>();
    }
    out[b] = (to_kilic & 1) ? g1_to_kilic(r) : r;
}

template <bool GLV> __device__ __forceinline__ void fb_walk_term(g1x_acc &acc, const g1a *table, uint64_t table_n, uint32_t c, uint32_t nwin, uint32_t D, uint64_t i,
                                                                const fr &k, uint32_t sg, bool phi) {
    uint32_t m[8];
    uint32_t sgn = sg;
    if (GLV) {
        const glv_halves h = glv_split_signed(k);
#pragma unroll
        for (int j = 0; j < 4; j++) { m[j] = phi ? h.k2[j] : h.k1[j]; m[4 + j] = 0; }
        sgn ^= phi ? h.neg2 : h.neg1;
    } else {
#pragma unroll
        for (int j = 0; j < 8; j++) m[j] = k.l[j];
    }
    auto bits = [&](uint32_t off) -> uint32_t {
        const uint32_t idx = off >> 5, sh = off & 31;
        if (idx >= (GLV ? 4u : 8u)) return 0u;
        uint64_t v = m[idx];
        if (idx + 1 < (GLV ? 4u : 8u)) v |= (uint64_t)m[idx + 1] << 32;
        return (uint32_t)(v >> sh) & ((1u << c) - 1u);
    };
    uint32_t raw = bits(0), carry, mag, ng;
    if (raw > D) { carry = 1; mag = (1u << c) - raw; ng = 1; } else { carry = 0; mag = raw; ng = 0; }
    g1a qn = table[((uint64_t)0 * table_n + i) * D + (mag ? mag - 1 : 0)];
#pragma nounroll
    for (uint32_t w = 0; w < nwin; w++) {
        g1a q = qn;
        const uint32_t cmag = mag, cng = ng ^ sgn;
        if (w + 1 < nwin) {
            raw = bits((w + 1) * c) + carry;
            if (raw > D) { carry = 1; mag = (1u << c) - raw; ng = 1; } else { carry = 0; mag = raw; ng = 0; }
            qn = table[((uint64_t)(w + 1) * table_n + i) * D + (mag ? mag - 1 : 0)];
        }
        if (cmag) {
            if (cng) q.y = neg<FpP>(q.y);
            acc.add(q);
        }
    }
}
template <bool GLV> __global__ __launch_bounds__(FB_BLOCK, 2) void k_fb_mul_vec(const g1a *table, uint64_t table_n, uint32_t c, uint32_t nwin, uint32_t D, const fr *scalars,
                                                         uint64_t i0, uint64_t cnt, uint64_t row, uint64_t total, g1j *out) {
    uint64_t t = blockIdx.x * (uint64_t)blockDim.x + threadIdx.x;
    if (t >= total) return;
    uint64_t jj = t % cnt, f = (t / cnt) % (table_n / row), b = t / (cnt * (table_n / row));
    uint64_t i = f * row + i0 + jj;
    const fr k = from_mont<FrP>(scalars[b * table_n + i]);
    g1x_acc acc; acc.init();
    if (GLV) { fb_walk_term<true>(acc, table, table_n, c, nwin, D, i, k, 0u, true); acc_apply_phi(acc); }
    fb_walk_term<GLV>(acc, table, table_n, c, nwin, D, i, k, 0u, false);
    out[t] = acc.to_jac();
}
struct fbp_slot { uint32_t w[39]; uint32_t inf; uint32_t pad; };
template <bool GLV> __global__ __launch_bounds__(64, 2) void k_fb_direct_pass1(const g1a *table, uint64_t table_n, uint32_t c, uint32_t nwin, uint32_t D, const fr *scalars, const fr *roots,
                                                           uint64_t W, uint32_t logn, uint32_t logR, uint64_t total, g1j *out) {
    __shared__ fbp_slot buf[64];
    const uint32_t tid = threadIdx.x;
    const uint64_t t = blockIdx.x * (uint64_t)blockDim.x + tid;
    const uint64_t n = 1ull << logn, R = 1ull << logR, cols = n >> logR;
    const uint32_t tt = (uint32_t)(t & (R - 1));
    const uint64_t u = (t >> logR) & (R - 1), jb = t >> (2 * logR), j = jb % cols, b = jb / cols;
    const bool live = t < total;
    g1jq_acc acc; acc.inf = true;
    if (live) {
        const uint64_t i = j + (uint64_t)tt * cols, e = ((uint64_t)tt * cols * u) & (n - 1);
        fr kmont = scalars[b * n + i];
        if (e) kmont = mul(kmont, roots[e * (W >> logn)]);
        const fr k = from_mont<FrP>(kmont);
        g1x_acc xa; xa.init();
        if (GLV) { fb_walk_term<true>(xa, table, table_n, c, nwin, D, i, k, 0u, true); acc_apply_phi(xa); }
        fb_walk_term<GLV>(xa, table, table_n, c, nwin, D, i, k, 0u, false);
        if (!xa.inf) { acc.v = g1jq_unpack(xa.to_jac()); acc.inf = false; }
    }
#define FBP_STORE(i_) do { _Pragma("unroll") for (int q_ = 0; q_ < 13; q_++) { buf[i_].w[q_] = acc.v.x.l[q_]; buf[i_].w[13 + q_] = acc.v.y.l[q_]; buf[i_].w[26 + q_] = acc.v.z.l[q_]; } \
                           buf[i_].inf = acc.inf ? 1u : 0u; } while (0)
    FBP_STORE(tid);
    __syncthreads();
#pragma nounroll
    for (uint32_t off = (uint32_t)R / 2; off >= 1; off >>= 1) {
        if (tt < off && !buf[tid + off].inf) {
            g1jq q;
#pragma unroll
            for (int i = 0; i < 13; i++) { q.x.l[i] = buf[tid + off].w[i]; q.y.l[i] = buf[tid + off].w[13 + i]; q.z.l[i] = buf[tid + off].w[26 + i]; }
            acc.add(q);
            FBP_STORE(tid);
        }
        __syncthreads();
    }
#undef FBP_STORE
    if (live && tt == 0) out[b * n + j * R + u] = acc.inf ? g1_inf() : g1jq_pack(acc.v);
}
void launch_fb_direct_pass1(hipStream_t s, const g1a *table, uint64_t table_n, uint32_t c, uint32_t nwin, const fr *scalars, const fr *roots, uint64_t W, uint64_t batch,
                            uint32_t logR, g1j *out, bool glv) {
    uint32_t logn = 0;
    while ((1ull << logn) < table_n) logn++;
    const uint64_t total = (batch * table_n) << logR, wgs = (total + 63) / 64;
    prof_begin(s, "fb_mul_vec");
    if (glv) hipLaunchKernelGGL(k_fb_direct_pass1<true>, dim3((uint32_t)wgs), dim3(64), wgs <= device_simds() ? 24 * 1024 : 0, s, table, table_n, c, nwin, 1u << (c - 1), scalars, roots, W, logn, logR,
                                total, out);
    else hipLaunchKernelGGL(k_fb_direct_pass1<false>, dim3((uint32_t)wgs), dim3(64), wgs <= device_simds() ? 24 * 1024 : 0, s, table, table_n, c, nwin, 1u << (c - 1), scalars, roots, W, logn, logR,
                            total, out);
    prof_end(s, "fb_mul_vec");
}

template <bool GLV> __global__ __launch_bounds__(FB_BLOCK, 2) void k_fb_mul_vec_dif2(const g1a *table, uint64_t table_n, uint32_t c, uint32_t nwin, uint32_t D, const fr *scalars,
                                                              const fr *roots, uint64_t W, uint64_t total, g1j *out) {
    uint64_t t = blockIdx.x * (uint64_t)blockDim.x + threadIdx.x;
    if (t >= total) return;
    const uint64_t N = table_n, q = N >> 2;
    const uint64_t i = t % q, o = (t / q) & 3u, b = t / N;
    const uint64_t rs = W / N;
    g1x_acc acc; acc.init();
#pragma nounroll
    for (uint32_t pass = GLV ? 0u : 1u; pass < 2; pass++) {
#pragma nounroll
        for (uint32_t term = 0; term < 4; term++) {
            const uint64_t pi = i + term * q;
            uint64_t e; uint32_t sg;
            if (o == 0) { e = 0; sg = 0; }
            else if (o == 1) { e = 2 * i; sg = term & 1u; }
            else if (o == 2) { e = i + ((term & 1u) ? q : 0); sg = term >> 1; }
            else { e = 3 * i + ((term & 1u) ? q : 0); sg = (term == 1 || term == 2) ? 1u : 0u; }
            fr kmont = scalars[b * N + pi];
            if (e) kmont = mul(kmont, roots[(e & (N - 1)) * rs]);
            const fr k = from_mont<FrP>(kmont);
            fb_walk_term<GLV>(acc, table, table_n, c, nwin, D, pi, k, sg, pass == 0);
        }
        if (GLV && pass == 0) acc_apply_phi(acc);
    }
    out[b * N + o * q + i] = acc.to_jac();
}
void launch_fb_mul_vec_dif2(hipStream_t s, const g1a *table, uint64_t table_n, uint32_t c, uint32_t nwin, const fr *scalars, const fr *roots, uint64_t W,
                            uint64_t batch, g1j *out, bool glv) {
    uint64_t total = batch * table_n;
    if (!total) return;
    prof_begin(s, "fb_mul_vec");
    if (glv) hipLaunchKernelGGL(k_fb_mul_vec_dif2<true>, dim3((uint32_t)((total + FB_BLOCK - 1) / FB_BLOCK)), dim3(FB_BLOCK), 0, s, table, table_n, c, nwin, 1u << (c - 1), scalars,
                                roots, W, total, out);
    else hipLaunchKernelGGL(k_fb_mul_vec_dif2<false>, dim3((uint32_t)((total + FB_BLOCK - 1) / FB_BLOCK)), dim3(FB_BLOCK), 0, s, table, table_n, c, nwin, 1u << (c - 1), scalars,
                            roots, W, total, out);
    prof_end(s, "fb_mul_vec");
}
template <bool GLV> __global__ __launch_bounds__(FB_BLOCK, 2) void k_fb_mul_vec_files(const g1a *table, uint64_t table_n, uint32_t c, uint32_t nwin, uint32_t D, const fr *scalars,
                                                               uint64_t i0, uint64_t cnt, uint64_t row, uint64_t total, g1j *out) {
    uint64_t t = blockIdx.x * (uint64_t)blockDim.x + threadIdx.x;
    if (t >= total) return;
    const uint64_t jj = t % cnt, b = t / cnt, nfiles = table_n / row;
    g1x_acc acc; acc.init();
#pragma nounroll
    for (uint32_t pass = GLV ? 0u : 1u; pass < 2; pass++) {
#pragma nounroll
        for (uint64_t f = 0; f < nfiles; f++) {
            const uint64_t i = f * row + i0 + jj;
            const fr k = from_mont<FrP>(scalars[b * table_n + i]);
            fb_walk_term<GLV>(acc, table, table_n, c, nwin, D, i, k, 0u, pass == 0);
        }
        if (GLV && pass == 0) acc_apply_phi(acc);
    }
    out[t] = acc.to_jac();
}
void launch_fb_mul_vec_files(hipStream_t s, const g1a *table, uint64_t table_n, uint32_t c, uint32_t nwin, const fr *scalars, uint64_t row, uint64_t j0,
                             uint64_t cnt, uint64_t batch, g1j *out, bool glv) {
    uint64_t total = batch * cnt;
    if (!total) return;
    prof_begin(s, "fb_mul_vec");
    if (glv) hipLaunchKernelGGL(k_fb_mul_vec_files<true>, dim3((uint32_t)((total + FB_BLOCK - 1) / FB_BLOCK)), dim3(FB_BLOCK), 0, s, table, table_n, c, nwin, 1u << (c - 1), scalars,
                                j0, cnt, row, total, out);
    else hipLaunchKernelGGL(k_fb_mul_vec_files<false>, dim3((uint32_t)((total + FB_BLOCK - 1) / FB_BLOCK)), dim3(FB_BLOCK), 0, s, table, table_n, c, nwin, 1u << (c - 1), scalars,
                            j0, cnt, row, total, out);
    prof_end(s, "fb_mul_vec");
}
void launch_fb_mul_vec(hipStream_t s, const g1a *table, uint64_t table_n, uint32_t c, uint32_t nwin, const fr *scalars, uint64_t row, uint64_t j0,
                       uint64_t cnt, uint64_t batch, g1j *out, bool glv) {
    uint64_t total = batch * (table_n / row) * cnt;
    if (!total) return;
    prof_begin(s, "fb_mul_vec");
    if (glv) hipLaunchKernelGGL(k_fb_mul_vec<true>, dim3((uint32_t)((total + FB_BLOCK - 1) / FB_BLOCK)), dim3(FB_BLOCK), 0, s, table, table_n, c, nwin, 1u << (c - 1), scalars,
                                j0, cnt, row, total, out);
    else hipLaunchKernelGGL(k_fb_mul_vec<false>, dim3((uint32_t)((total + FB_BLOCK - 1) / FB_BLOCK)), dim3(FB_BLOCK), 0, s, table, table_n, c, nwin, 1u << (c - 1), scalars,
                            j0, cnt, row, total, out);
    prof_end(s, "fb_mul_vec");
}

uint64_t device_simd_lanes() {
    static std::atomic<uint64_t> lanes_of_device[64];
    int dev = 0;
    (void)hipGetDevice(&dev);
    std::atomic<uint64_t> &slot = lanes_of_device[dev >= 0 && dev < 64 ? dev : 0];
    uint64_t lanes = slot.load(std::memory_order_relaxed);
    if (!lanes) {
        int cus = 256;
        if (hipDeviceGetAttribute(&cus, hipDeviceAttributeMultiprocessorCount, dev) != hipSuccess) { (void)hipGetLastError(); cus = 256; }
        lanes = (uint64_t)(cus > 0 ? cus : 256) * 4 * 64;
        slot.store(lanes, std::memory_order_relaxed);
    }
    return lanes;
}
static uint32_t fb_blocks_per_blob(uint64_t n, uint64_t batch, uint32_t *wsplit = nullptr) {
    uint64_t lanes = knobs::fb_lanes() ? knobs::fb_lanes() : 2 * device_simd_lanes();
    if (lanes < FB_ACC_BLOCK) lanes = FB_ACC_BLOCK;
    uint64_t target = lanes / FB_ACC_BLOCK;
    uint64_t bpb = target / (batch ? batch : 1);
    uint32_t split = 1;
    while (split < 8 && (batch ? batch : 1) * n * split * 2 <= lanes) split *= 2;
    if (wsplit) *wsplit = split;
    uint64_t maxb = (n * split + FB_ACC_BLOCK - 1) / FB_ACC_BLOCK;
    if (bpb > maxb) bpb = maxb;
    if (bpb < 1) bpb = 1;
    return (uint32_t)bpb;
}
size_t fb_partials_bytes(uint64_t n, uint64_t batch) { return (((size_t)std::max(fb_blocks_per_blob(n, batch), fb_blocks_per_blob(2 * n, batch)) * batch * sizeof(fb_partial)) + 15) / 16 * 16; }

void launch_fb_msm(hipStream_t s, const g1a *table, uint64_t table_n, uint32_t c, uint32_t nwin, const fr *scalars, uint64_t sc_stride, uint64_t n,
                   uint64_t batch, void *partials, g1j *out, bool to_kilic, bool glv, bool projective) {
    if (!batch) return;
    const int fin = (to_kilic ? 1 : 0) | (projective ? 2 : 0);
    uint32_t split = 1;
    uint32_t bpb = fb_blocks_per_blob(glv ? 2 * n : n, batch, &split);
    if (split > nwin) split = nwin;
    prof_begin(s, "fb_accumulate");
    if (glv) {
        if (split > 1) hipLaunchKernelGGL(k_fb_accumulate_glv<true>, dim3((uint32_t)(batch * bpb)), dim3(FB_ACC_BLOCK), 0, s, table, table_n, c, nwin, 1u << (c - 1), scalars, sc_stride, n,
                                          bpb, split, (fb_partial *)partials);
        else hipLaunchKernelGGL(k_fb_accumulate_glv<false>, dim3((uint32_t)(batch * bpb)), dim3(FB_ACC_BLOCK), 0, s, table, table_n, c, nwin, 1u << (c - 1), scalars, sc_stride, n, bpb,
                                1u, (fb_partial *)partials);
    } else if (split > 1) hipLaunchKernelGGL(k_fb_accumulate<true>, dim3((uint32_t)(batch * bpb)), dim3(FB_ACC_BLOCK), 0, s, table, table_n, c, nwin, 1u << (c - 1), scalars, sc_stride, n,
                                      bpb, split, (fb_partial *)partials);
    else hipLaunchKernelGGL(k_fb_accumulate<false>, dim3((uint32_t)(batch * bpb)), dim3(FB_ACC_BLOCK), 0, s, table, table_n, c, nwin, 1u << (c - 1), scalars, sc_stride, n, bpb,
                            1u, (fb_partial *)partials);
    prof_end(s, "fb_accumulate");
    if (bpb <= FB_FINISH_LANES_MAX) hipLaunchKernelGGL(k_fb_finish_lanes, dim3((uint32_t)((batch + 63) / 64)), dim3(64), 0, s, (const fb_partial *)partials, bpb, batch, out, fin);
    else hipLaunchKernelGGL(k_fb_finish, dim3((uint32_t)batch), dim3(256), 0, s, (const fb_partial *)partials, bpb, batch, out, fin);
}
hipError_t launch_fb_build(hipStream_t s, const g1a *pts, uint64_t n, uint32_t c, uint32_t nwin, g1a *table) {
    uint32_t D = 1u << (c - 1);
    g1j *rows_j = nullptr; g1a *rows = nullptr; fp *ztmp = nullptr, *ptmp = nullptr;
    uint64_t lanes_all = (uint64_t)nwin * n;
    hipError_t e;
    if ((e = hipMallocAsync((void **)&rows_j, lanes_all * sizeof(g1j), s)) != hipSuccess) return e;
    if ((e = hipMallocAsync((void **)&rows, lanes_all * sizeof(g1a), s)) != hipSuccess) { hipFreeAsync(rows_j, s); return e; }
    launch_msm_window_table(s, pts, n, c, nwin, rows_j, rows);
    uint64_t per_win = n * D * sizeof(fp);
    uint32_t slab = (uint32_t)((1ull << 30) / (per_win ? per_win : 1));
    if (slab < 1) slab = 1;
    if (slab > nwin) slab = nwin;
    if ((e = hipMallocAsync((void **)&ztmp, (uint64_t)slab * per_win, s)) != hipSuccess) { hipFreeAsync(rows_j, s); hipFreeAsync(rows, s); return e; }
    if ((e = hipMallocAsync((void **)&ptmp, (uint64_t)slab * per_win, s)) != hipSuccess) { hipFreeAsync(rows_j, s); hipFreeAsync(rows, s); hipFreeAsync(ztmp, s); return e; }
    for (uint32_t w0 = 0; w0 < nwin; w0 += slab) {
        uint32_t ws = (w0 + slab <= nwin) ? slab : nwin - w0;
        uint64_t lanes = (uint64_t)ws * n;
        uint32_t S = D;
        while (S > 64 && lanes * (D / S) < (1ull << 20)) S >>= 1;
        dim3 g((uint32_t)((lanes * (D / S) + FB_BLOCK - 1) / FB_BLOCK)), b(FB_BLOCK);
        hipLaunchKernelGGL(k_fb_build_pass1, g, b, 0, s, rows + (uint64_t)w0 * n, lanes, D, S, table + (uint64_t)w0 * n * D, ztmp);
        hipLaunchKernelGGL(k_fb_build_pass2, g, b, 0, s, lanes, D, S, table + (uint64_t)w0 * n * D, ztmp, ptmp);
    }
    hipFreeAsync(rows_j, s); hipFreeAsync(rows, s); hipFreeAsync(ztmp, s); hipFreeAsync(ptmp, s);
    return hipGetLastError();
}

__global__ __launch_bounds__(MSM_ACC_BLOCK, 2) void k_msm_window_rows(const g1a *pts, uint64_t n, uint32_t c, uint32_t nwin, g1j *tmp) {
    uint64_t i = blockIdx.x * (uint64_t)blockDim.x + threadIdx.x;
    if (i >= n) return;
    g1j q = to_jac(pts[i]);
#pragma nounroll
    for (uint32_t w = 0; w < nwin; w++) {
        tmp[(uint64_t)w * n + i] = q;
#pragma nounroll
        for (uint32_t j = 0; j < c; j++) q = g1_dbl(q);
    }
}
void launch_msm_window_table(hipStream_t s, const g1a *pts, uint64_t n, uint32_t c, uint32_t nwin, g1j *tmp, g1a *out) {
    if (!n) return;
    hipLaunchKernelGGL(k_msm_window_rows, dim3((uint32_t)((n + MSM_ACC_BLOCK - 1) / MSM_ACC_BLOCK)), dim3(MSM_ACC_BLOCK), 0, s, pts, n, c, nwin, tmp);
    launch_g1_to_affine(s, tmp, out, n * nwin);
}

}
```

### go-kzg_amd/csrc/knobs.hpp

```cpp
#pragma once
#include <limits.h>
#include <stdint.h>
#include <stdlib.h>
#include <string.h>

namespace kzg {

enum { FAULT_RCCL = 1, FAULT_RCCL_CORRUPT = 2, FAULT_PEER = 4, FAULT_PEER_CORRUPT = 8, FAULT_RCCL_HANG = 16, FAULT_PEER_HANG = 32, FAULT_PEER_STUCK = 64, FAULT_RCCL_BLOCK = 128, FAULT_RCCL_INIT_BLOCK = 256 };

namespace knobs {

enum class g1_fft_mode { by_size, direct, radix2 };
enum class g1_mul_mode { by_shape, regular, wnaf };
enum class fr_fft_mode { by_size, radix2, shared };
enum class zero_poly_mode { by_size, direct, tree };
enum class msm_reduce_mode { by_batch, scan, chunks };
enum class transcript_mode { by_count, host, device };
enum class pairing_mode { by_count, lane, wave };
enum class combine_mode { by_count, never, always };
enum class transport_mode { by_devices, rccl, host, peer };
struct opt_gb { bool set; double gb; };

inline bool is(const char *e, const char *word) { return e && !strcmp(e, word); }
inline bool starts(const char *e, char c) { return e && e[0] == c; }
inline bool list_has(const char *e, const char *word) {
    const size_t n = strlen(word);
    for (const char *at = e; e && (at = strstr(at, word)); at += n)
        if ((at == e || at[-1] == ',') && (at[n] == 0 || at[n] == ',')) return true;
    return false;
}
inline zero_poly_mode zero_poly_of(const char *e) { return is(e, "direct") ? zero_poly_mode::direct : is(e, "tree") ? zero_poly_mode::tree : zero_poly_mode::by_size; }
inline double positive_or(const char *e, double dflt) { const double v = e ? atof(e) : 0.0; return v > 0.0 ? v : dflt; }
inline unsigned multi_fault_of(const char *e) {
    if (!e) return 0;
    return (list_has(e, "rccl") ? FAULT_RCCL : 0) | (list_has(e, "rccl-corrupt") ? FAULT_RCCL_CORRUPT : 0) | (list_has(e, "peer") ? FAULT_PEER : 0) |
           (list_has(e, "peer-corrupt") ? FAULT_PEER_CORRUPT : 0) | (list_has(e, "rccl-hang") ? FAULT_RCCL_HANG : 0) |
           (list_has(e, "rccl-block") ? FAULT_RCCL_BLOCK : 0) |
           (list_has(e, "rccl-init-block") ? FAULT_RCCL_INIT_BLOCK : 0) |
           (list_has(e, "peer-hang") ? FAULT_PEER_HANG : 0) |
           (list_has(e, "peer-stuck") ? FAULT_PEER_HANG | FAULT_PEER_STUCK : 0);
}

#define KZG_KNOB_ONCE(type, fn, name, expr)                   \
    inline type parse_##fn(const char *e) { return expr; }    \
    inline type fn() { static type const v = parse_##fn(getenv(name)); return v; }
#define KZG_KNOB_PER_CALL(type, fn, name, expr)               \
    inline type parse_##fn(const char *e) { return expr; }    \
    inline type fn() { return parse_##fn(getenv(name)); }
#define KZG_KNOB_PER_HANDLE KZG_KNOB_PER_CALL

KZG_KNOB_ONCE(bool, fb_glv, "KZG_HIP_FB_GLV", !is(e, "0"))
KZG_KNOB_ONCE(bool, coalesce, "KZG_HIP_COALESCE", !starts(e, '0'))
KZG_KNOB_ONCE(bool, upload_ramp, "KZG_HIP_UPLOAD_RAMP", !starts(e, '0'))
KZG_KNOB_ONCE(bool, lincomb_promote, "KZG_HIP_LINCOMB_PROMOTE", !starts(e, '0'))
KZG_KNOB_ONCE(bool, stream_cache, "KZG_HIP_STREAM_CACHE", !starts(e, '0'))
KZG_KNOB_ONCE(bool, g1_direct_coop, "KZG_HIP_G1_DIRECT_COOP", !starts(e, '0'))
KZG_KNOB_ONCE(bool, coop_inv, "KZG_HIP_COOP_INV", !starts(e, '0'))
KZG_KNOB_ONCE(bool, fk20_pass1, "KZG_HIP_FK20_PASS1", !starts(e, '0'))
KZG_KNOB_ONCE(bool, fk20_fuse, "KZG_HIP_FK20_FUSE", !starts(e, '0'))
KZG_KNOB_ONCE(bool, fk20_pad, "KZG_HIP_FK20_PAD", !starts(e, '0'))
KZG_KNOB_PER_CALL(bool, eth_prove_overlap, "KZG_HIP_ETH_PROVE_OVERLAP", !starts(e, '0'))
KZG_KNOB_ONCE(bool, coalesce_trace, "KZG_HIP_COALESCE_TRACE", e != nullptr)
KZG_KNOB_PER_CALL(bool, coalesce_stats, "KZG_HIP_COALESCE_STATS", e != nullptr)
KZG_KNOB_ONCE(bool, eth_quotient_one, "KZG_HIP_ETH_QUOTIENT", is(e, "one"))
KZG_KNOB_ONCE(bool, sha256_portable, "KZG_HIP_SHA256", is(e, "portable"))

KZG_KNOB_ONCE(g1_fft_mode, g1_fft, "KZG_HIP_G1_FFT", !e ? g1_fft_mode::by_size : e[0] == 'd' ? g1_fft_mode::direct : g1_fft_mode::radix2)
KZG_KNOB_ONCE(int, g1_quad, "KZG_HIP_G1_QUAD", !e ? -1 : e[0] == '0' ? 0 : e[0] == '2' ? 2 : 1)
KZG_KNOB_ONCE(g1_mul_mode, g1_mul, "KZG_HIP_G1_MUL", starts(e, 'r') ? g1_mul_mode::regular : starts(e, 'w') ? g1_mul_mode::wnaf : g1_mul_mode::by_shape)
KZG_KNOB_ONCE(fr_fft_mode, fr_fft, "KZG_HIP_FR_FFT", is(e, "radix2") ? fr_fft_mode::radix2 : is(e, "shared") ? fr_fft_mode::shared : fr_fft_mode::by_size)
KZG_KNOB_ONCE(zero_poly_mode, zero_poly_once, "KZG_HIP_ZERO_POLY", zero_poly_of(e))
KZG_KNOB_PER_CALL(zero_poly_mode, zero_poly_per_call, "KZG_HIP_ZERO_POLY", zero_poly_of(e))
KZG_KNOB_ONCE(msm_reduce_mode, msm_reduce, "KZG_HIP_MSM_REDUCE", is(e, "chunks") ? msm_reduce_mode::chunks : is(e, "scan") ? msm_reduce_mode::scan : msm_reduce_mode::by_batch)
KZG_KNOB_ONCE(int, msm_seg, "KZG_HIP_MSM_SEG", e ? atoi(e) : -1)
KZG_KNOB_PER_CALL(transcript_mode, eth_transcript, "KZG_HIP_ETH_TRANSCRIPT", is(e, "host") ? transcript_mode::host : is(e, "device") ? transcript_mode::device : transcript_mode::by_count)
KZG_KNOB_PER_CALL(pairing_mode, pairing, "KZG_HIP_PAIRING", is(e, "lane") ? pairing_mode::lane : is(e, "wave") ? pairing_mode::wave : pairing_mode::by_count)
KZG_KNOB_PER_CALL(combine_mode, verify_combine, "KZG_HIP_VERIFY_COMBINE", is(e, "never") ? combine_mode::never : is(e, "always") ? combine_mode::always : combine_mode::by_count)
KZG_KNOB_PER_CALL(int, multi_fft, "KZG_HIP_MULTI_FFT", !e ? -1 : is(e, "sharded") ? 1 : 0)
KZG_KNOB_PER_HANDLE(transport_mode, multi_transport, "KZG_HIP_MULTI_TRANSPORT", !e ? transport_mode::by_devices : is(e, "rccl") ? transport_mode::rccl : is(e, "host") ? transport_mode::host : transport_mode::peer)
KZG_KNOB_PER_HANDLE(unsigned, multi_fault, "KZG_HIP_MULTI_FAULT", multi_fault_of(e))
KZG_KNOB_ONCE(const char *, rccl_lib, "KZG_HIP_RCCL_LIB", e)

KZG_KNOB_ONCE(uint32_t, lincomb_promote_after, "KZG_HIP_LINCOMB_PROMOTE_AFTER", (uint32_t)(!e ? 2 : atol(e) < 1 ? 1 : atol(e) > 1000 ? 1000 : atol(e)))
KZG_KNOB_ONCE(uint64_t, fb_lanes, "KZG_HIP_FB_LANES", e ? strtoull(e, nullptr, 10) : 0ull)
KZG_KNOB_ONCE(uint64_t, eth_stage_rows, "KZG_HIP_ETH_STAGE_ROWS", e ? (uint64_t)atol(e) : 0ull)
KZG_KNOB_PER_CALL(uint64_t, verify_combine_rows, "KZG_HIP_VERIFY_COMBINE_ROWS", e && strtoull(e, nullptr, 10) >= 1 ? strtoull(e, nullptr, 10) : 0ull)
KZG_KNOB_PER_CALL(double, eth_verify_chunk_mb, "KZG_HIP_ETH_VERIFY_CHUNK_MB", positive_or(e, 4096.0))
KZG_KNOB_PER_CALL(double, eth_prove_chunk_mb, "KZG_HIP_ETH_PROVE_CHUNK_MB", positive_or(e, 4096.0))
KZG_KNOB_PER_CALL(double, recover_chunk_mb, "KZG_HIP_RECOVER_CHUNK_MB", positive_or(e, 2048.0))
KZG_KNOB_PER_CALL(opt_gb, fb_budget_gb, "KZG_HIP_FB_BUDGET_GB", (opt_gb{e != nullptr, e ? atof(e) : 0.0}))
KZG_KNOB_PER_CALL(opt_gb, points_fb_budget_gb, "KZG_HIP_POINTS_FB_BUDGET_GB", (opt_gb{e != nullptr, e ? atof(e) : 0.0}))
KZG_KNOB_PER_CALL(opt_gb, fk20_fb_budget_gb, "KZG_HIP_FK20_FB_BUDGET_GB", (opt_gb{e != nullptr, e ? atof(e) : 0.0}))
KZG_KNOB_PER_HANDLE(long, multi_probe_timeout_ms, "KZG_HIP_MULTI_PROBE_TIMEOUT_MS", e && atol(e) >= 10 && atol(e) <= 600000 ? atol(e) : 10000)
KZG_KNOB_PER_HANDLE(long, coalesce_us, "KZG_HIP_COALESCE_US", e ? atol(e) : 150)
KZG_KNOB_PER_HANDLE(long, coalesce_spin_us, "KZG_HIP_COALESCE_SPIN_US", e ? atol(e) : 40)
KZG_KNOB_PER_CALL(int, coalesce_sim_max_bufs, "KZG_COALESCE_SIM_MAX_BUFS", e ? atoi(e) : INT_MAX)

#undef KZG_KNOB_ONCE
#undef KZG_KNOB_PER_CALL
#undef KZG_KNOB_PER_HANDLE

inline int parse_coalesce_exec(const char *e, int dflt, int max) { return !e ? dflt : atoi(e) < 1 ? 1 : atoi(e) > max ? max : atoi(e); }
inline int coalesce_exec(int dflt, int max) { return parse_coalesce_exec(getenv("KZG_HIP_COALESCE_EXEC"), dflt, max); }
inline int parse_coalesce_per_batch(const char *e, int dflt) { return !e ? dflt : atoi(e) < 1 ? 1 : atoi(e); }
inline int coalesce_per_batch(int dflt) { return parse_coalesce_per_batch(getenv("KZG_HIP_COALESCE_PER_BATCH"), dflt); }

}
}
```

Baseline: 104,200 commitments/s.

## Add shared single-window fixed-base table layout for large commit batches

Adds a second fixed-base layout in which one table of 2^(c-1) multiples per setup point is shared by all windows. It uses larger window sizes (fewer windows) within the same memory budget, at the cost of a Horner-style doubling chain in the finish step. Scalars are first decomposed into signed GLV digits in a workspace. An accumulate kernel then walks the phi and plain digit streams per window against the shared table, and a finish kernel combines windows with c doublings each. For batches at or above a threshold (2048 by default), the per-window table is freed or skipped in favour of the shared one when it needs fewer additions. This adds digit workspace traffic, doublings, a table rebuild and a one-time device sync.

```diff
diff --git a/go-kzg_amd/csrc/capi_common.hpp b/go-kzg_amd/csrc/capi_common.hpp
--- a/go-kzg_amd/csrc/capi_common.hpp
+++ b/go-kzg_amd/csrc/capi_common.hpp
@@ -75,7 +75,11 @@
     g1a *d_secret_a = nullptr;
     g1a *d_fixed = nullptr;
     msm_plan fixed_plan{};
+    g1a *d_shared = nullptr;
+    msm_plan shared_plan{};
+    bool shared_first = false;
     double budget_gb = -1.0;
+    double resolved_budget_gb = -1.0;
     std::atomic<bool> projective{false};
     hipStream_t copy_stream = nullptr;
     hipEvent_t copy_done[2] = {nullptr, nullptr};
@@ -233,7 +237,8 @@
 int ensure_fixed_table(kzg_hip_kzg *ks, hipStream_t);
 const void *host_mapped_pointer(const void *host, size_t bytes);
 int h2d_copy(void *dst, const void *src, size_t bytes, hipStream_t s);
-int commit_rows(kzg_hip_kzg *ks, hipStream_t s, const fr *d_sc, uint64_t n, uint64_t batch, g1j *d_out, uint64_t sc_stride = 0, bool to_kilic = true);
+int commit_rows(kzg_hip_kzg *ks, hipStream_t s, const fr *d_sc, uint64_t n, uint64_t batch, g1j *d_out, uint64_t sc_stride = 0, bool to_kilic = true, bool may_share = false);
+int prepare_shared_table(kzg_hip_kzg *ks, uint64_t batch);
 double table_budget_gb(knobs::opt_gb env, double cap_gb, double headroom_gb);
 int lincomb_points_rows(kzg_hip_points *pts, hipStream_t s, const fr *d_sc, uint64_t n, uint64_t batch, g1j *d_out, uint64_t sc_stride = 0, bool holds_mu = false);
 int lincomb_points_coalesced(kzg_hip_points *pts, const void *scalars_fr, uint64_t n, void *out_g1);
diff --git a/go-kzg_amd/csrc/capi_kzg.hip b/go-kzg_amd/csrc/capi_kzg.hip
--- a/go-kzg_amd/csrc/capi_kzg.hip
+++ b/go-kzg_amd/csrc/capi_kzg.hip
@@ -31,7 +31,7 @@
     if (!ks) return;
     hipSetDevice(ks->fs->device);
     hipDeviceSynchronize();
-    hipFree(ks->d_secret); hipFree(ks->d_secret_a); hipFree(ks->d_fixed);
+    hipFree(ks->d_secret); hipFree(ks->d_secret_a); hipFree(ks->d_fixed); hipFree(ks->d_shared);
     if (ks->copy_stream) { stream_cache_disown(ks->copy_stream); hipStreamDestroy(ks->copy_stream); }
     for (int i = 0; i < 2; i++) if (ks->copy_done[i]) hipEventDestroy(ks->copy_done[i]);
     (void)hipGetLastError();
@@ -54,16 +54,23 @@
 #ifndef FB_DEFAULT_BUDGET_GB
 #define FB_DEFAULT_BUDGET_GB 110.0
 #endif
-uint32_t fb_windows_glv(uint32_t c) { return (128 + c - 1) / c; }
+uint32_t fb_windows_glv(uint32_t c) { return fb_shared_windows(c); }
 bool fb_glv_enabled() { return knobs::fb_glv(); }
+static double fb_plan_bytes(const msm_plan &p) { return (double)p.nwin * (double)p.table_n * (double)p.nb * sizeof(g1a); }
+static double fb_handle_budget_gb(kzg_hip_kzg *ks) {
+    if (ks->budget_gb >= 0.0) return ks->budget_gb;
+    if (!((ks->d_fixed || ks->d_shared) && ks->resolved_budget_gb >= 0.0)) ks->resolved_budget_gb = table_budget_gb(knobs::fb_budget_gb(), FB_DEFAULT_BUDGET_GB, 24.0);
+    return ks->resolved_budget_gb;
+}
+static bool fb_window_size_skipped(uint32_t c, bool glv) { return glv ? (c == 14) : (c == 15); }
 int ensure_fixed_table(kzg_hip_kzg *ks, hipStream_t) {
     if (ks->d_fixed || ks->fixed_plan.c == 0xffffffffu) return KZG_HIP_OK;
     hipStream_t s = ks->fs->stream;
-    double budget_gb = ks->budget_gb >= 0.0 ? ks->budget_gb : table_budget_gb(knobs::fb_budget_gb(), FB_DEFAULT_BUDGET_GB, 24.0);
+    const double budget_gb = fb_handle_budget_gb(ks) - (ks->d_shared ? (double)ks->shared_plan.table_n * (double)ks->shared_plan.nb * sizeof(g1a) / 1e9 : 0.0);
     if (ks->n_setup < 64) { ks->fixed_plan.c = 0xffffffffu; return KZG_HIP_OK; }
     const bool glv = fb_glv_enabled();
     for (uint32_t c = 16; c >= 5; c--) {
-        if (glv ? (c == 14) : (c == 15)) continue;
+        if (fb_window_size_skipped(c, glv)) continue;
         const uint32_t nwin = glv ? fb_windows_glv(c) : fb_windows(c);
         double bytes = (double)nwin * (double)ks->n_setup * (double)(1u << (c - 1)) * sizeof(g1a);
         if (bytes > budget_gb * 1e9) continue;
@@ -82,10 +89,99 @@
     return KZG_HIP_OK;
 }
 
-int commit_rows(kzg_hip_kzg *ks, hipStream_t s, const fr *d_sc, uint64_t n, uint64_t batch, g1j *d_out, uint64_t sc_stride, bool to_kilic) {
-    CHK(ensure_fixed_table(ks, s));
+#ifndef FB_SHARED_MIN_BATCH
+#define FB_SHARED_MIN_BATCH 2048
+#endif
+#ifndef FB_SHARED_CHUNK
+#define FB_SHARED_CHUNK 4096
+#endif
+#ifndef FB_SHARED_MIN_BATCH_REPLACED
+#define FB_SHARED_MIN_BATCH_REPLACED 256
+#endif
+static uint32_t fb_shared_pick(uint64_t n_setup, double bytes, uint32_t below = 20) {
+    for (uint32_t c = below - 1; c >= 5; c--) {
+        if (c > 5 && fb_shared_windows(c - 1) == fb_shared_windows(c)) continue;
+        if ((double)n_setup * (double)(1u << (c - 1)) * sizeof(g1a) <= bytes) return c;
+    }
+    return 0;
+}
+static uint32_t fb_plan_additions(const msm_plan &p) { return p.glv ? 2 * p.nwin : p.nwin; }
+static uint32_t fb_windows_additions_at(uint64_t n_setup, double bytes, bool glv) {
+    for (uint32_t c = 16; c >= 5; c--) {
+        if (fb_window_size_skipped(c, glv)) continue;
+        const uint32_t nwin = glv ? fb_windows_glv(c) : fb_windows(c);
+        if ((double)nwin * (double)n_setup * (double)(1u << (c - 1)) * sizeof(g1a) <= bytes) return glv ? 2 * nwin : nwin;
+    }
+    return UINT32_MAX;
+}
+static uint64_t fb_shared_threshold(const kzg_hip_kzg *ks) {
+    if (const uint64_t forced = knobs::fb_shared_min_batch()) return forced;
+    if (knobs::fb_layout() == knobs::fb_layout_mode::shared) return 1;
+    return ks->shared_first ? FB_SHARED_MIN_BATCH_REPLACED : FB_SHARED_MIN_BATCH;
+}
+static bool fb_shared_build(kzg_hip_kzg *ks, double bytes, uint32_t fewer_than) {
+    hipStream_t s = ks->fs->stream;
+    for (uint32_t c = fb_shared_pick(ks->n_setup, bytes); c && 2 * fb_shared_windows(c) < fewer_than; c = fb_shared_pick(ks->n_setup, bytes, c)) {
+        msm_plan p{};
+        p.c = c; p.nwin = fb_shared_windows(c); p.nb = 1u << (c - 1); p.ngroups = 1; p.fixed = 1; p.glv = 1; p.table_n = ks->n_setup;
+        g1a *tab = nullptr;
+        if (hipMalloc((void **)&tab, (size_t)ks->n_setup * p.nb * sizeof(g1a)) != hipSuccess) { (void)hipGetLastError(); continue; }
+        hipError_t e = launch_fb_build_shared(s, ks->d_secret_a, ks->n_setup, c, tab);
+        if (e == hipSuccess) e = hipStreamSynchronize(s);
+        if (e != hipSuccess) { (void)hipGetLastError(); hipFree(tab); continue; }
+        ks->d_shared = tab; ks->shared_plan = p;
+        return true;
+    }
+    return false;
+}
+static int ensure_shared_table(kzg_hip_kzg *ks) {
+    if (ks->d_shared || ks->shared_plan.c == 0xffffffffu) return KZG_HIP_OK;
+    if (ks->n_setup < 64 || !fb_glv_enabled()) { ks->shared_plan.c = 0xffffffffu; return KZG_HIP_OK; }
+    const double budget = fb_handle_budget_gb(ks) * 1e9;
+    if (ks->d_fixed) {
+        if (fb_shared_build(ks, budget - fb_plan_bytes(ks->fixed_plan), fb_plan_additions(ks->fixed_plan))) return KZG_HIP_OK;
+        const uint32_t c = fb_shared_pick(ks->n_setup, budget);
+        if (!c || 2 * fb_shared_windows(c) >= fb_plan_additions(ks->fixed_plan)) { ks->shared_plan.c = 0xffffffffu; return KZG_HIP_OK; }
+        HIPCHK(hipDeviceSynchronize());
+        HIPCHK(hipFree(ks->d_fixed));
+        ks->d_fixed = nullptr; ks->fixed_plan = msm_plan{};
+    }
+    if (fb_shared_build(ks, budget, fb_windows_additions_at(ks->n_setup, budget, true))) ks->shared_first = true;
+    else ks->shared_plan.c = 0xffffffffu;
+    return KZG_HIP_OK;
+}
+int prepare_shared_table(kzg_hip_kzg *ks, uint64_t batch) {
+    if (knobs::fb_layout() == knobs::fb_layout_mode::windows) return KZG_HIP_OK;
+    {
+        dev_guard g(ks->fs);
+        if (ks->d_shared || ks->shared_plan.c == 0xffffffffu || batch < fb_shared_threshold(ks)) return KZG_HIP_OK;
+    }
+    std::unique_lock<std::shared_mutex> tl(ks->tab_mu);
+    dev_guard g(ks->fs);
+    return ensure_shared_table(ks);
+}
+
+int commit_rows(kzg_hip_kzg *ks, hipStream_t s, const fr *d_sc, uint64_t n, uint64_t batch, g1j *d_out, uint64_t sc_stride, bool to_kilic, bool may_share) {
+    if (!sc_stride) sc_stride = n;
+    bool share = may_share && ks->d_shared && knobs::fb_layout() != knobs::fb_layout_mode::windows && batch >= fb_shared_threshold(ks);
+    if (!share) {
+        CHK(ensure_fixed_table(ks, s));
+        share = may_share && !ks->d_fixed && ks->d_shared && knobs::fb_layout() != knobs::fb_layout_mode::windows;
+    }
+    if (share) {
+        const uint64_t piece = batch < FB_SHARED_CHUNK ? batch : FB_SHARED_CHUNK;
+        dtmp<uint8_t> d_ws(s);
+        if (d_ws.alloc(fb_shared_workspace_bytes(n, piece, ks->shared_plan.c)) == KZG_HIP_OK) {
+            const bool projective = to_kilic && ks->projective.load(std::memory_order_relaxed);
+            for (uint64_t b0 = 0; b0 < batch; b0 += piece)
+                launch_fb_msm_shared(s, ks->d_shared, ks->shared_plan.c, d_sc + b0 * sc_stride, sc_stride, n, batch - b0 < piece ? batch - b0 : piece, d_ws.p, d_out + b0, to_kilic, projective);
+            HIPCHK(hipGetLastError());
+            return KZG_HIP_OK;
+        }
+        (void)hipGetLastError();
+        CHK(ensure_fixed_table(ks, s));
+    }
     bool fixed = ks->d_fixed != nullptr;
-    if (!sc_stride) sc_stride = n;
     msm_plan p = fixed ? ks->fixed_plan : classic_plan(ks->n_setup);
     if (!fixed && !msm_index_range_ok(p, n)) return KZG_HIP_ERR_TOO_WIDE;
     size_t ws_main = fixed ? fb_partials_bytes(n, batch) : msm_workspace_bytes(p, n, batch);
@@ -100,8 +196,10 @@
     if (!ks || !(gb >= 0.0)) return KZG_HIP_ERR_BAD_ARG;
     std::unique_lock<std::shared_mutex> tl(ks->tab_mu);
     dev_guard g(ks->fs);
-    if (ks->d_fixed) { HIPCHK(hipDeviceSynchronize()); HIPCHK(hipFree(ks->d_fixed)); ks->d_fixed = nullptr; }
-    ks->fixed_plan = msm_plan{};
+    if (ks->d_fixed || ks->d_shared) HIPCHK(hipDeviceSynchronize());
+    if (ks->d_fixed) { HIPCHK(hipFree(ks->d_fixed)); ks->d_fixed = nullptr; }
+    if (ks->d_shared) { HIPCHK(hipFree(ks->d_shared)); ks->d_shared = nullptr; }
+    ks->fixed_plan = msm_plan{}; ks->shared_plan = msm_plan{}; ks->shared_first = false; ks->resolved_budget_gb = -1.0;
     ks->budget_gb = gb;
     return KZG_HIP_OK;
 }
@@ -111,8 +209,9 @@
     if (n > ks->n_setup) return KZG_HIP_ERR_LEN_MISMATCH;
     if (!batch) return KZG_HIP_OK;
     if (n == 0 || !d_coeffs_fr) return KZG_HIP_ERR_BAD_ARG;
+    CHK(prepare_shared_table(ks, batch));
     dev_guard g(ks->fs);
-    return commit_rows(ks, (hipStream_t)stream, (const fr *)d_coeffs_fr, n, batch, (g1j *)d_out_g1);
+    return commit_rows(ks, (hipStream_t)stream, (const fr *)d_coeffs_fr, n, batch, (g1j *)d_out_g1, 0, true, true);
 }
 namespace {
 std::mutex g_reg_mu;
@@ -194,19 +293,23 @@
     if (!batch) return KZG_HIP_OK;
     if (n == 0) { for (uint64_t b = 0; b < batch; b++) set_inf_image((uint8_t *)out_g1 + b * sizeof(g1j)); return KZG_HIP_OK; }
     if (!coeffs_fr) return KZG_HIP_ERR_BAD_ARG;
+    uint64_t chunk = batch >= 1024 ? 512 : (batch >= 512 ? 256 : batch);
+    if (n * sizeof(fr) < (64u << 10)) chunk = batch;
+    const fr *mapped = nullptr;
+    { dev_select sel(ks->fs); mapped = (const fr *)host_mapped_pointer(coeffs_fr, (size_t)n * batch * sizeof(fr)); }
+    CHK(prepare_shared_table(ks, mapped ? batch : chunk));
     dev_guard g(ks->fs);
     hipStream_t s = ks->fs->stream;
     dtmp<fr> d_sc(s); dtmp<g1j> d_out(s);
     CHK(d_out.alloc(batch));
-    if (const fr *mapped = (const fr *)host_mapped_pointer(coeffs_fr, (size_t)n * batch * sizeof(fr))) {
-        CHK(commit_rows(ks, s, mapped, n, batch, d_out.p));
+    if (mapped) {
+        CHK(commit_rows(ks, s, mapped, n, batch, d_out.p, 0, true, true));
         HIPCHK(hipMemcpyAsync(out_g1, d_out.p, batch * sizeof(g1j), hipMemcpyDeviceToHost, s));
         HIPCHK(hipStreamSynchronize(s));
         return KZG_HIP_OK;
     }
     CHK(d_sc.alloc(n * batch));
-    uint64_t chunk = batch >= 1024 ? 512 : (batch >= 512 ? 256 : batch);
-    if (chunk < batch && n * sizeof(fr) >= (64u << 10)) {
+    if (chunk < batch) {
         if (!ks->copy_stream) {
             HIPCHK(hipStreamCreateWithFlags(&ks->copy_stream, hipStreamNonBlocking));
             stream_cache_own(ks->copy_stream);
@@ -224,11 +327,11 @@
             CHK(h2d_copy(d_sc.p + b0 * n, (const fr *)coeffs_fr + b0 * n, n * cnt * sizeof(fr), ks->copy_stream));
             HIPCHK(hipEventRecord(ks->copy_done[slot], ks->copy_stream));
             HIPCHK(hipStreamWaitEvent(s, ks->copy_done[slot], 0));
-            CHK(commit_rows(ks, s, d_sc.p + b0 * n, n, cnt, d_out.p + b0));
+            CHK(commit_rows(ks, s, d_sc.p + b0 * n, n, cnt, d_out.p + b0, 0, true, true));
         }
     } else {
         CHK(h2d_copy(d_sc.p, coeffs_fr, n * batch * sizeof(fr), s));
-        CHK(commit_rows(ks, s, d_sc.p, n, batch, d_out.p));
+        CHK(commit_rows(ks, s, d_sc.p, n, batch, d_out.p, 0, true, true));
     }
     HIPCHK(hipMemcpyAsync(out_g1, d_out.p, batch * sizeof(g1j), hipMemcpyDeviceToHost, s));
     HIPCHK(hipStreamSynchronize(s));
@@ -462,9 +565,9 @@
 
 int kzg_hip_kzg_table_info(kzg_hip_kzg *ks, uint32_t *window_bits, uint32_t *windows, uint64_t *table_bytes) {
     if (!ks || !window_bits || !windows || !table_bytes) return KZG_HIP_ERR_BAD_ARG;
-    bool have = ks->d_fixed != nullptr;
-    *window_bits = have ? ks->fixed_plan.c : 0; *windows = have ? ks->fixed_plan.nwin : 0;
-    *table_bytes = have ? (uint64_t)ks->fixed_plan.nwin * ks->fixed_plan.table_n * ks->fixed_plan.nb * sizeof(g1a) : 0;
+    const msm_plan *p = ks->d_fixed ? &ks->fixed_plan : ks->d_shared ? &ks->shared_plan : nullptr;
+    *window_bits = p ? p->c : 0; *windows = p ? p->nwin : 0;
+    *table_bytes = p ? (uint64_t)(ks->d_fixed ? p->nwin : 1) * p->table_n * p->nb * sizeof(g1a) : 0;
     return KZG_HIP_OK;
 }
 int kzg_hip_kzg_set_projective_outputs(kzg_hip_kzg *ks, int on) {
@@ -473,6 +576,7 @@
     return KZG_HIP_OK;
 }
 uint32_t kzg_hip_kzg_table_additions(kzg_hip_kzg *ks) {
-    if (!ks || !ks->d_fixed) return 0;
+    if (!ks || (!ks->d_fixed && !ks->d_shared)) return 0;
+    if (!ks->d_fixed) return 2 * ks->shared_plan.nwin;
     return ks->fixed_plan.glv ? 2 * ks->fixed_plan.nwin : ks->fixed_plan.nwin;
 }
diff --git a/go-kzg_amd/csrc/internal.hpp b/go-kzg_amd/csrc/internal.hpp
--- a/go-kzg_amd/csrc/internal.hpp
+++ b/go-kzg_amd/csrc/internal.hpp
@@ -107,6 +107,11 @@
 hipError_t launch_fb_build(hipStream_t s, const g1a *pts, uint64_t n, uint32_t c, uint32_t nwin, g1a *table);
 void launch_fb_msm(hipStream_t s, const g1a *table, uint64_t table_n, uint32_t c, uint32_t nwin, const fr *scalars, uint64_t sc_stride, uint64_t n,
                    uint64_t batch, void *partials, g1j *out, bool to_kilic, bool glv = false, bool projective = false);
+inline uint32_t fb_shared_windows(uint32_t c) { return (128 + c - 1) / c; }
+size_t fb_shared_workspace_bytes(uint64_t n, uint64_t batch, uint32_t c);
+hipError_t launch_fb_build_shared(hipStream_t s, const g1a *pts, uint64_t n, uint32_t c, g1a *table);
+void launch_fb_msm_shared(hipStream_t s, const g1a *table, uint32_t c, const fr *scalars, uint64_t sc_stride, uint64_t n, uint64_t batch, void *workspace, g1j *out,
+                          bool to_kilic, bool projective);
 
 void launch_fb_mul_vec(hipStream_t s, const g1a *table, uint64_t table_n, uint32_t c, uint32_t nwin, const fr *scalars, uint64_t row, uint64_t j0,
                        uint64_t cnt, uint64_t batch, g1j *out, bool glv = false);
diff --git a/go-kzg_amd/csrc/k_msm.hip b/go-kzg_amd/csrc/k_msm.hip
--- a/go-kzg_amd/csrc/k_msm.hip
+++ b/go-kzg_amd/csrc/k_msm.hip
@@ -313,37 +313,45 @@
     if (live && c == 0) fb_partial_store(((fb_partial *)(ws + b * per_blob + gsum_off))[g], S);
 }
 
+__device__ __forceinline__ void quad_horner_finish(const fb_partial *sums, uint32_t ngroups, uint32_t ndbl, uint32_t per_group, bool live, uint32_t role, g1j *dst, int fin) {
+    g1x_acc acc; acc.init();
+    acc.v = g1xq_from_affine(g1a_inf());
+#pragma nounroll
+    for (uint32_t g = ngroups; g-- > 0;) {
+#pragma nounroll
+        for (uint32_t j = 0; j < ndbl; j++) {
+            g1xq d = acc.v;
+            quad_xyzz_dbl(d, role);
+            if (!acc.inf) acc.v = d;
+        }
+#pragma nounroll
+        for (uint32_t j = 0; j < per_group; j++) {
+            const fb_partial &pj = sums[(uint64_t)g * per_group + j];
+            const bool winf = !live || pj.inf != 0;
+            g1xq w;
+            if (winf) w = acc.v; else fb_partial_load(pj, w);
+            quad_acc_add(acc, w, winf, role);
+        }
+    }
+    {
+        const bool own = live && role == 0;
+        const g1x px = g1xq_pack(acc.v);
+        const fp i = wave_inv_any(mul(px.zz, px.zzz), own && !acc.inf && !(fin & 2));
+        if (own) {
+            g1j r;
+            if (acc.inf) r = g1_inf();
+            else if (fin & 2) r = g1x_to_jac(px);
+            else { r.x = mul(px.x, mul(i, px.zzz)); r.y = mul(px.y, mul(i, px.zz)); r.z = one<FpP>(); }
+            *dst = (fin & 1) ? g1_to_kilic(r) : r;
+        }
+    }
+}
 __global__ __launch_bounds__(256) void k_msm_combine(uint8_t *ws, size_t per_blob, size_t gsum_off, uint32_t ngroups, uint64_t batch, g1j *out, int to_kilic) {
     const uint32_t role = threadIdx.x & 3u;
     const uint64_t b = blockIdx.x * 64ull + (threadIdx.x >> 2);
     const bool live = b < batch;
     const fb_partial *gsum = (const fb_partial *)(ws + (live ? b : 0) * per_blob + gsum_off);
-    g1x_acc acc; acc.init();
-    acc.v = g1xq_from_affine(g1a_inf());
-#pragma nounroll
-    for (uint32_t g = ngroups; g-- > 0;) {
-#pragma nounroll
-        for (uint32_t j = 0; j < 8; j++) {
-            g1xq d = acc.v;
-            quad_xyzz_dbl(d, role);
-            if (!acc.inf) acc.v = d;
-        }
-        const bool winf = !live || gsum[g].inf != 0;
-        g1xq w;
-        if (winf) w = acc.v; else fb_partial_load(gsum[g], w);
-        quad_acc_add(acc, w, winf, role);
-    }
-    {
-        const bool own = live && role == 0;
-        const g1x px = g1xq_pack(acc.v);
-        const fp i = wave_inv_any(mul(px.zz, px.zzz), own && !acc.inf);
-        if (own) {
-            g1j r;
-            if (acc.inf) r = g1_inf();
-            else { r.x = mul(px.x, mul(i, px.zzz)); r.y = mul(px.y, mul(i, px.zz)); r.z = one<FpP>(); }
-            out[b] = to_kilic ? g1_to_kilic(r) : r;
-        }
-    }
+    quad_horner_finish(gsum, ngroups, 8, 1, live, role, out + (live ? b : 0), to_kilic ? 1 : 0);
 }
 
 void launch_msm(hipStream_t s, const msm_plan &p, const g1a *table, const fr *scalars, uint64_t sc_stride, uint64_t n, uint64_t batch, void *workspace, g1j *out,
@@ -682,6 +690,96 @@
     out[b] = (to_kilic & 1) ? g1_to_kilic(r) : r;
 }
 
+#define FB_DIGIT_MAG 0xfffffu
+__global__ __launch_bounds__(256) void k_fb_digits(const fr *scalars, uint64_t sc_stride, uint64_t n, uint64_t batch, uint32_t c, uint32_t W, uint32_t *digits) {
+    const uint64_t t = blockIdx.x * 256ull + threadIdx.x;
+    if (t >= n * batch) return;
+    const uint64_t blob = t / n, i = t % n;
+    const glv_halves h = glv_split_signed(from_mont<FrP>(scalars[blob * sc_stride + i]));
+    const uint32_t D = 1u << (c - 1);
+#pragma unroll
+    for (uint32_t half = 0; half < 2; half++) {
+        uint32_t m[4];
+#pragma unroll
+        for (int j = 0; j < 4; j++) m[j] = half ? h.k1[j] : h.k2[j];
+        const uint32_t sgn = (half ? h.neg1 : h.neg2) ? 1u : 0u;
+        uint32_t *dst = digits + ((blob * 2 + half) * W) * n + i;
+        uint32_t carry = 0;
+#pragma nounroll
+        for (uint32_t w = 0; w < W; w++) {
+            const uint32_t raw = mag_bits(m, w * c, c) + carry;
+            uint32_t mag, ng;
+            if (raw > D) { carry = 1; mag = (1u << c) - raw; ng = 1; } else { carry = 0; mag = raw; ng = 0; }
+            dst[(uint64_t)w * n] = mag ? (mag | ((ng ^ sgn) << 31)) : 0u;
+        }
+    }
+}
+__global__ __launch_bounds__(FB_ACC_BLOCK, FB_ACC_WAVES) void k_fb_accumulate_shared(const g1a *table, uint32_t D, uint32_t W, uint32_t Q, const uint32_t *digits, uint64_t n,
+                                                                                   uint32_t blocks_per_blob, fb_partial *partials) {
+    __shared__ fb_partial buf[64];
+    const uint32_t tid = threadIdx.x, role = tid & 3u, quad = tid >> 2;
+    const uint64_t blob = blockIdx.x / blocks_per_blob; const uint32_t blk = blockIdx.x % blocks_per_blob;
+    const bool live = quad < W * Q;
+    const uint32_t w = live ? quad / Q : 0u;
+    const uint32_t LW = 4 * Q;
+    g1x_acc acc; acc.init();
+    if (live) {
+        const uint64_t stride = (uint64_t)blocks_per_blob * LW;
+        const uint64_t i0 = (uint64_t)blk * LW + (tid - w * LW);
+        const uint64_t cnt = i0 < n ? (n - i0 + stride - 1) / stride : 0;
+        const uint32_t *dphi = digits + ((blob * 2) * W + w) * n, *dplain = dphi + (uint64_t)W * n;
+        const uint64_t K = 2 * cnt;
+        if (K) {
+            uint32_t wc = dphi[i0];
+            g1a qn = table[i0 * D + ((wc & FB_DIGIT_MAG) ? (wc & FB_DIGIT_MAG) - 1 : 0)];
+            uint32_t wn = cnt > 1 ? dphi[i0 + stride] : dplain[i0];
+#pragma nounroll
+            for (uint64_t k = 0; k < K; k++) {
+                const g1a q0 = qn;
+                const uint32_t cur = wc;
+                wc = wn;
+                if (k + 1 < K) {
+                    const uint64_t i1 = i0 + (k + 1 < cnt ? k + 1 : k + 1 - cnt) * stride;
+                    qn = table[i1 * D + ((wc & FB_DIGIT_MAG) ? (wc & FB_DIGIT_MAG) - 1 : 0)];
+                }
+                if (k + 2 < K) wn = k + 2 < cnt ? dphi[i0 + (k + 2) * stride] : dplain[i0 + (k + 2 - cnt) * stride];
+                if (k == cnt && !acc.inf) acc.v.x = mulq(acc.v.x, unpackq(glv_beta()));
+                if (cur & FB_DIGIT_MAG) {
+                    g1a q = q0;
+                    if (cur >> 31) q.y = neg<FpP>(q.y);
+                    acc.add(q);
+                }
+            }
+        }
+    }
+    if (acc.inf) acc.v = g1xq_from_affine(g1a_inf());
+    const uint32_t ainf = acc.inf ? 1u : 0u;
+    g1x_acc col;
+    { uint32_t vi; quad_point_bcast<0>(col.v, vi, acc.v, ainf); col.inf = vi != 0; }
+    { g1xq v; uint32_t vi; quad_point_bcast<1>(v, vi, acc.v, ainf); quad_tree_add(col, v, vi != 0, role); }
+    { g1xq v; uint32_t vi; quad_point_bcast<2>(v, vi, acc.v, ainf); quad_tree_add(col, v, vi != 0, role); }
+    { g1xq v; uint32_t vi; quad_point_bcast<3>(v, vi, acc.v, ainf); quad_tree_add(col, v, vi != 0, role); }
+    if (col.inf) col.v = g1xq_from_affine(g1a_inf());
+    if (role == 0) fb_partial_store(buf[quad], col);
+    __syncthreads();
+    const uint32_t base = live ? w * Q : quad;
+    g1x_acc sum;
+    fb_partial_load(buf[base], sum.v); sum.inf = buf[base].inf != 0;
+#pragma nounroll
+    for (uint32_t j = 1; j < Q; j++) {
+        const fb_partial &src = buf[live ? base + j : quad];
+        g1xq v; fb_partial_load(src, v);
+        quad_tree_add(sum, v, !live || src.inf != 0, role);
+    }
+    if (live && quad == base && role == 0) fb_partial_store(partials[(blob * W + w) * blocks_per_blob + blk], sum);
+}
+__global__ __launch_bounds__(256) void k_fb_finish_shared(const fb_partial *partials, uint32_t c, uint32_t W, uint32_t blocks_per_blob, uint64_t batch, g1j *out, int fin) {
+    const uint32_t role = threadIdx.x & 3u;
+    const uint64_t b = blockIdx.x * 64ull + (threadIdx.x >> 2);
+    const bool live = b < batch;
+    quad_horner_finish(partials + (live ? b : 0) * W * blocks_per_blob, W, c, blocks_per_blob, live, role, out + (live ? b : 0), fin);
+}
+
 template <bool GLV> __device__ __forceinline__ void fb_walk_term(g1x_acc &acc, const g1a *table, uint64_t table_n, uint32_t c, uint32_t nwin, uint32_t D, uint64_t i,
                                                                 const fr &k, uint32_t sg, bool phi) {
     uint32_t m[8];
@@ -912,6 +1010,41 @@
     prof_end(s, "fb_accumulate");
     if (bpb <= FB_FINISH_LANES_MAX) hipLaunchKernelGGL(k_fb_finish_lanes, dim3((uint32_t)((batch + 63) / 64)), dim3(64), 0, s, (const fb_partial *)partials, bpb, batch, out, fin);
     else hipLaunchKernelGGL(k_fb_finish, dim3((uint32_t)batch), dim3(256), 0, s, (const fb_partial *)partials, bpb, batch, out, fin);
+}
+static uint32_t fb_shared_blocks_per_blob(uint64_t n, uint64_t batch, uint32_t W) {
+    const uint32_t LW = 4 * (64 / W);
+    const uint64_t maxb = (n + LW - 1) / LW;
+    const uint64_t bpb = fb_blocks_per_blob(2 * n, batch);
+    return (uint32_t)(bpb > maxb ? maxb : bpb);
+}
+static size_t fb_shared_digit_bytes(uint64_t n, uint64_t batch, uint32_t W) { return (((size_t)batch * 2 * W * n * sizeof(uint32_t)) + 15) / 16 * 16; }
+size_t fb_shared_workspace_bytes(uint64_t n, uint64_t batch, uint32_t c) {
+    const uint32_t W = fb_shared_windows(c);
+    return fb_shared_digit_bytes(n, batch, W) + (((size_t)fb_shared_blocks_per_blob(n, batch, W) * W * batch * sizeof(fb_partial)) + 15) / 16 * 16;
+}
+void launch_fb_msm_shared(hipStream_t s, const g1a *table, uint32_t c, const fr *scalars, uint64_t sc_stride, uint64_t n, uint64_t batch, void *workspace, g1j *out,
+                          bool to_kilic, bool projective) {
+    if (!batch) return;
+    const uint32_t W = fb_shared_windows(c), Q = 64 / W;
+    const uint32_t bpb = fb_shared_blocks_per_blob(n, batch, W);
+    uint32_t *digits = (uint32_t *)workspace;
+    fb_partial *partials = (fb_partial *)((uint8_t *)workspace + fb_shared_digit_bytes(n, batch, W));
+    hipLaunchKernelGGL(k_fb_digits, dim3((uint32_t)((n * batch + 255) / 256)), dim3(256), 0, s, scalars, sc_stride, n, batch, c, W, digits);
+    prof_begin(s, "fb_accumulate");
+    hipLaunchKernelGGL(k_fb_accumulate_shared, dim3((uint32_t)(batch * bpb)), dim3(FB_ACC_BLOCK), 0, s, table, 1u << (c - 1), W, Q, digits, n, bpb, partials);
+    prof_end(s, "fb_accumulate");
+    hipLaunchKernelGGL(k_fb_finish_shared, dim3((uint32_t)((batch + 63) / 64)), dim3(256), 0, s, (const fb_partial *)partials, c, W, bpb, batch, out,
+                       (to_kilic ? 1 : 0) | (projective ? 2 : 0));
+}
+hipError_t launch_fb_build_shared(hipStream_t s, const g1a *pts, uint64_t n, uint32_t c, g1a *table) {
+    const uint64_t D = 1ull << (c - 1);
+    uint64_t slice = (1ull << 30) / (D * sizeof(fp));
+    if (slice < 1) slice = 1;
+    for (uint64_t i0 = 0; i0 < n; i0 += slice) {
+        const hipError_t e = launch_fb_build(s, pts + i0, n - i0 < slice ? n - i0 : slice, c, 1, table + i0 * D);
+        if (e != hipSuccess) return e;
+    }
+    return hipSuccess;
 }
 hipError_t launch_fb_build(hipStream_t s, const g1a *pts, uint64_t n, uint32_t c, uint32_t nwin, g1a *table) {
     uint32_t D = 1u << (c - 1);
diff --git a/go-kzg_amd/csrc/knobs.hpp b/go-kzg_amd/csrc/knobs.hpp
--- a/go-kzg_amd/csrc/knobs.hpp
+++ b/go-kzg_amd/csrc/knobs.hpp
@@ -19,6 +19,7 @@
 enum class pairing_mode { by_count, lane, wave };
 enum class combine_mode { by_count, never, always };
 enum class transport_mode { by_devices, rccl, host, peer };
+enum class fb_layout_mode { by_batch, windows, shared };
 struct opt_gb { bool set; double gb; };
 
 inline bool is(const char *e, const char *word) { return e && !strcmp(e, word); }
@@ -76,6 +77,7 @@
 KZG_KNOB_PER_CALL(transcript_mode, eth_transcript, "KZG_HIP_ETH_TRANSCRIPT", is(e, "host") ? transcript_mode::host : is(e, "device") ? transcript_mode::device : transcript_mode::by_count)
 KZG_KNOB_PER_CALL(pairing_mode, pairing, "KZG_HIP_PAIRING", is(e, "lane") ? pairing_mode::lane : is(e, "wave") ? pairing_mode::wave : pairing_mode::by_count)
 KZG_KNOB_PER_CALL(combine_mode, verify_combine, "KZG_HIP_VERIFY_COMBINE", is(e, "never") ? combine_mode::never : is(e, "always") ? combine_mode::always : combine_mode::by_count)
+KZG_KNOB_PER_CALL(fb_layout_mode, fb_layout, "KZG_HIP_FB_LAYOUT", is(e, "windows") ? fb_layout_mode::windows : is(e, "shared") ? fb_layout_mode::shared : fb_layout_mode::by_batch)
 KZG_KNOB_PER_CALL(int, multi_fft, "KZG_HIP_MULTI_FFT", !e ? -1 : is(e, "sharded") ? 1 : 0)
 KZG_KNOB_PER_HANDLE(transport_mode, multi_transport, "KZG_HIP_MULTI_TRANSPORT", !e ? transport_mode::by_devices : is(e, "rccl") ? transport_mode::rccl : is(e, "host") ? transport_mode::host : transport_mode::peer)
 KZG_KNOB_PER_HANDLE(unsigned, multi_fault, "KZG_HIP_MULTI_FAULT", multi_fault_of(e))
@@ -84,6 +86,7 @@
 KZG_KNOB_ONCE(uint32_t, lincomb_promote_after, "KZG_HIP_LINCOMB_PROMOTE_AFTER", (uint32_t)(!e ? 2 : atol(e) < 1 ? 1 : atol(e) > 1000 ? 1000 : atol(e)))
 KZG_KNOB_ONCE(uint64_t, fb_lanes, "KZG_HIP_FB_LANES", e ? strtoull(e, nullptr, 10) : 0ull)
 KZG_KNOB_ONCE(uint64_t, eth_stage_rows, "KZG_HIP_ETH_STAGE_ROWS", e ? (uint64_t)atol(e) : 0ull)
+KZG_KNOB_PER_CALL(uint64_t, fb_shared_min_batch, "KZG_HIP_FB_SHARED_MIN_BATCH", e && strtoull(e, nullptr, 10) >= 1 ? strtoull(e, nullptr, 10) : 0ull)
 KZG_KNOB_PER_CALL(uint64_t, verify_combine_rows, "KZG_HIP_VERIFY_COMBINE_ROWS", e && strtoull(e, nullptr, 10) >= 1 ? strtoull(e, nullptr, 10) : 0ull)
 KZG_KNOB_PER_CALL(double, eth_verify_chunk_mb, "KZG_HIP_ETH_VERIFY_CHUNK_MB", positive_or(e, 4096.0))
 KZG_KNOB_PER_CALL(double, eth_prove_chunk_mb, "KZG_HIP_ETH_PROVE_CHUNK_MB", positive_or(e, 4096.0))
```

Result: faster. 113,700 commitments/s (median of 6 runs) (+9.1%).
